# StandeHaas/Hydrodynamic-Limits-of-Active-Particle-Systems-with-Mean-Field-Interactions

Measured on AMD Instinct MI355X. Metric: particle-steps/sec at N=1e5, higher is better.
Workload: dtype f64; 1 GPU; BASELINE config 2: N=100000 particles, L=200000 sites, K=1, reflecting walls, sigma=0.005 (4001-tap table), beta=0.7, dt=0.0125, exclusion on; method=tiles

## Files before the change

hydrodynamic-limits-of-active-particle-systems-with-mean-field-interactions_amd/csrc/aps_hip.hip:

```cpp

#include <hip/hip_runtime.h>
#include <hip/hip_ext.h>
#include <dlfcn.h>
#include <unistd.h>
#include <rccl/rccl.h>
#include <algorithm>
#include <cmath>
#include <cstdint>
#include <cstdio>
#include <cstdlib>
#include <cstring>
#include <numeric>
#include <string>
#include <vector>

#include "aps.h"
#include "aps_common.hpp"
#include "dev_mem.hpp"

namespace {

constexpr uint32_t POS_MASK = 0x07FFFFFFu;
constexpr uint32_t SPIN_BIT = 1u << 27;
constexpr uint32_t BOUND_BIT = 1u << 28;
// ... 1718 lines not shown
#endif
#undef TS_CASE
#undef TS_PICK
}
const void *ts_kernel(bool periodic, bool tab, int RS, bool k1, bool f32 = false) {
    return f32 ? ts_kernel_f<true>(periodic, tab, RS, k1) : ts_kernel_f<false>(periodic, tab, RS, k1);
}
constexpr int TS_RS_CHOICES[] = {1, 2, 3, 4, 5, 6, 7, 8};

int ts_wbytes(const aps_handle *h) { return h->f32 ? 4 : 8; }

void ts_choose_geometry(aps_handle *h) {
    const int L = h->p.L;
    h->ts_RS = 1;
    double best = 1e300;
    for (int rs : TS_RS_CHOICES) {
        const int own = 64 * rs - 4;
        const double wgs = (double)(((int64_t)L + own - 1) / own) * h->E;
        const double miss = std::fabs(wgs - 2.4 * 256.0);
        if (miss < best) { best = miss; h->ts_RS = rs; }
    }
    if ((double)(((int64_t)L + 507) / 508) * h->E > 3.0 * 256.0)
        h->ts_RS = !h->f32 ? 4 : 7;
    int own_even = 0;
    if (h->world == 1 && h->model.field_mode && 3 * h->p.K <= 32 && !(h->p.K == 1 && h->model.immobilize && h->model.k_exit > 0.0)) {
        int cus = 0;
        if (hipDeviceGetAttribute(&cus, hipDeviceAttributeMultiprocessorCount, h->p.device) != hipSuccess || cus <= 0) { (void)hipGetLastError(); cus = 256; }
        const int64_t target = 2LL * cus / std::max(h->E, 1);
        if (target >= 1) {
            const int own = (int)((L + target - 1) / target), rs = (own + 4 + 63) / 64;
            if (own >= 124 && rs <= 8) { h->ts_RS = rs; own_even = own; }
        }
    }
    if (const char *env = std::getenv("APS_TS_R")) { const int r = std::atoi(env); if (ts_kernel(false, true, r, true)) { h->ts_RS = r; own_even = 0; } }
    h->ts_own = own_even ? own_even : 64 * h->ts_RS - 4;
    if (const char *env = std::getenv("APS_TS_OWN")) { const int o = std::atoi(env); if (o >= 32 * h->ts_RS && o <= 64 * h->ts_RS - 4) h->ts_own = o; }
    while (h->ts_own > 32 * h->ts_RS && L > h->ts_own && (L % h->ts_own == 1 || L % h->ts_own == 2)) h->ts_own -= 1;
    h->ts_ntile = (L + h->ts_own - 1) / h->ts_own;
    h->ts_dcap = (int)std::max<int64_t>(2, std::min<int64_t>(2LL * h->p.K * h->ts_own, 2 * h->p.n_particles));
    h->ts_table_in_lds = ts_lds_layout(h->tlen, true, h->ts_RS, h->ts_own, h->p.K, ts_wbytes(h)).total <= 160 * 1024;
    h->ts_lo = (int)((int64_t)h->rank * h->ts_ntile / h->world);
    h->ts_hi = (int)((int64_t)(h->rank + 1) * h->ts_ntile / h->world);
    h->own_lo = h->ts_lo * h->ts_own;
    h->own_hi = std::min(L, h->ts_hi * h->ts_own);
    h->ts_reach = h->model.field_mode ? (h->tlen + 2 + h->ts_own - 1) / h->ts_own : 0;
    h->ts_kx = 1;
    if (h->world > 1) {
        const int reach = std::max(h->ts_reach, 1);
        int own_min = h->ts_ntile, own_max = 0;
        for (int r = 0; r < h->world; ++r) {
            const int n = (int)((int64_t)(r + 1) * h->ts_ntile / h->world) - (int)((int64_t)r * h->ts_ntile / h->world);
            own_min = std::min(own_min, n); own_max = std::max(own_max, n);
        }
        auto fits = [&](int k) { return k * reach <= own_min && own_max + 2 * (k - 1) * reach <= h->ts_ntile; };
        const int64_t budget = std::max<int64_t>(768 / std::max(h->E, 1), (int64_t)own_max + own_max / 4);
        int k = 1;
        while (k < 8 && fits(k + 1) && own_max + 2 * k * reach <= budget) ++k;
        if (h->p.halo_interval > 0) k = h->p.halo_interval;
        else if (const char *env = std::getenv("APS_HALO_INTERVAL")) k = std::max(1, std::atoi(env));
        h->ts_kx = k;
    }
}

TileArgs tile_args(aps_handle *h, bool field_only) {
    TileArgs a{};
    const int par = (int)(h->step & 1), out = field_only ? par : par ^ 1;
    a.L = h->p.L; a.K = h->p.K; a.tlen = h->tlen; a.own = h->ts_own; a.ntile = h->ts_ntile; a.dcap = h->ts_dcap; a.par = par;
    a.dense = h->ntt_on ? h->d_ntt_csig : nullptr; a.dense_rt = h->ntt.Rt; a.dense_m = h->ntt.lc; a.periodic = h->p.periodic;
    a.dense_org = h->ntt.org; a.dense_shard = h->world > 1 ? 1 : 0;
    a.dense_lo = h->world > 1 ? h->own_lo : 0; a.dense_hi = h->world > 1 ? h->own_hi : h->p.L;
    a.tile_lo = h->ts_lo; a.field_only = field_only ? 1 : 0; a.field_mode = h->model.field_mode; a.ens_base = h->model.ens_base; a.E = h->E;
    a.seed_lo = h->model.seed_lo; a.seed_hi = h->model.seed_hi;
    a.model = h->d_model; a.rare = h->d_rare;
    a.ws_in = h->f32 ? (const void *)h->d_wsi[par] : (const void *)h->d_wsb[par];
    a.ws_out = h->f32 ? (void *)h->d_wsi[out] : (void *)h->d_wsb[out];
    a.cell_in = h->d_cell[par]; a.cell_out = h->d_cell[par ^ 1];
    a.dcnt_in = h->d_tdcnt[par]; a.dep_in = h->d_tdep[par]; a.dcnt_out = h->d_tdcnt[par ^ 1]; a.dep_out = h->d_tdep[par ^ 1];
    a.gpart_in = h->d_gpart[par]; a.gpart_out = h->d_gpart[par ^ 1];
    a.stepw = h->d_stepw; a.beta = h->d_beta; a.anchor = h->d_anchor;
    return a;
}

int launch_tile_step(aps_handle *h, bool field_only = false) {
    int rc = field_only ? APS_OK : prof_mark(h, KIND_TILE_STEP);
    if (rc) return rc;
    TileArgs a = tile_args(h, field_only);
    if (h->ntt_on) {
        if (field_only) return fail(h, APS_ERR_STATE, "tiles, convolution: no deposits are ever pending");
        a.tile_lo = 0;
        const dim3 grid((unsigned)td_tiles(a.dense_hi - a.dense_lo), (unsigned)h->E), block(FU_THREADS);
        const void *fn = h->f32 ? (h->p.K == 1 ? reinterpret_cast<const void *>(&tile_dense<true, true>) : reinterpret_cast<const void *>(&tile_dense<false, true>))
                                : (h->p.K == 1 ? reinterpret_cast<const void *>(&tile_dense<true, false>) : reinterpret_cast<const void *>(&tile_dense<false, false>));
        void *args[] = {(void *)&a};
        if (h->profiling && h->prof_dispatch) HIP_TRY(h, hipExtLaunchKernel(fn, grid, block, args, td_lds_bytes(h->p.K), h->stream, h->k_start, h->k_stop, 0));
        else HIP_TRY(h, hipLaunchKernel(fn, grid, block, args, td_lds_bytes(h->p.K), h->stream));
        h->slots_dirty = true; h->field_pending = true; h->ws_view_stale = true;
        return APS_OK;
    }
    int t0 = h->ts_lo, t1 = h->ts_hi;
    if (h->world > 1) {
        if (!field_only && h->halo_age >= h->ts_kx) return fail(h, APS_ERR_STATE, "tiles, sharded: the halo exchange of the last step is missing");
        const int g = (h->ts_kx - 1 - std::min(h->halo_age, h->ts_kx - 1)) * h->ts_reach + (field_only ? 1 : 0);
        t0 = h->p.periodic ? t0 - g : std::max(0, t0 - g);
        t1 = h->p.periodic ? t1 + g : std::min(h->ts_ntile, t1 + g);
    }
    const void *fn = ts_kernel(h->p.periodic != 0, h->ts_table_in_lds, h->ts_RS, h->p.K == 1, h->f32);
    const size_t lds = ts_lds_layout(h->tlen, h->ts_table_in_lds, h->ts_RS, h->ts_own, h->p.K, ts_wbytes(h)).total;
    const void *table_ptr = h->f32 ? (const void *)h->d_table_i : (const void *)h->d_table;
    void *args[] = {(void *)&a, (void *)&table_ptr};
    struct Piece { int lo, hi; } pieces[3];
    int np = 0;
    if (t0 < 0) pieces[np++] = {t0 + h->ts_ntile, h->ts_ntile};
    pieces[np++] = {std::max(t0, 0), std::min(t1, h->ts_ntile)};
    if (t1 > h->ts_ntile) pieces[np++] = {0, t1 - h->ts_ntile};
    for (int i = 0; i < np; ++i) {
        if (pieces[i].hi <= pieces[i].lo) continue;
        a.tile_lo = pieces[i].lo;
        const dim3 grid((unsigned)(pieces[i].hi - pieces[i].lo), (unsigned)h->E), block(FU_THREADS);
        if (!field_only && h->profiling && h->prof_dispatch)
            HIP_TRY(h, hipExtLaunchKernel(fn, grid, block, args, lds, h->stream, h->k_start, h->k_stop, 0));
        else
            HIP_TRY(h, hipLaunchKernel(fn, grid, block, args, lds, h->stream));
    }
    if (!field_only) { h->slots_dirty = true; h->field_pending = true; }
    h->ws_view_stale = true;
    return APS_OK;
}

int launch_ntt_conv(aps_handle *h) {
    const int out = (int)((h->step & 1) ^ 1);
    const NttPlan &pl = h->ntt;
    const unsigned tiles = (unsigned)(((size_t)1 << pl.m) / NTT_TILE);
    const dim3 grid_e(tiles, 2u, (unsigned)(h->E * pl.nb)), grid_p(tiles, 2u, (unsigned)(h->E * pl.np * pl.nb)), block(NTT_THREADS);
    int *const clr = pl.nb > 1 ? h->d_ntt_csig : nullptr;
    void *ws = h->f32 ? (void *)h->d_wsi[out] : (void *)h->d_wsb[out];
    int rc;
    const bool timed = h->profiling && h->prof_dispatch;
#define NTT_STRIDED(AXIS, INV, NP_, GRID, A_, CSIG, WS, FLAG) do { if ((rc = prof_mark(h, KIND_NTT))) return rc; \
        ntt_launch_strided<AXIS, INV, NP_>(A_, GRID, block, h->stream, h->k_start, h->k_stop, timed, pl, h->d_ntt_sig, CSIG, WS, FLAG); } while (0)
#define NTT_ENDS(AXIS, INV, A_, CSIG, WS) do { if (pl.np == 2) NTT_STRIDED(2, INV, 2, grid_e, A_, CSIG, WS, 1); else NTT_STRIDED(AXIS, INV, 1, grid_e, A_, CSIG, WS, 1); } while (0)
    if (h->ntt_fused) {
        NTT_ENDS(2, false, pl.a2, h->d_ntt_csig, nullptr);
        if ((rc = prof_mark(h, KIND_NTT))) return rc;
        APS_K(h, ntt_mid, dim3(1u << pl.a2, 2u, (unsigned)(h->E * pl.np * pl.nb)), dim3(NTT_MID_THREADS), NTT_MID_LDS, pl, h->d_ntt_sig);
        NTT_ENDS(2, true, pl.a2, clr, ws);
        HIP_TRY(h, hipGetLastError());
        h->field_pending = false;
        return APS_OK;
    }
    if (pl.a2 > 0) {
        NTT_ENDS(2, false, pl.a2, h->d_ntt_csig, nullptr);
        NTT_STRIDED(1, false, 1, grid_p, pl.a1, (int *)nullptr, nullptr, 0);
    } else NTT_ENDS(1, false, pl.a1, h->d_ntt_csig, nullptr);
    if ((rc = prof_mark(h, KIND_NTT))) return rc;
    APS_K(h, (ntt_contig<false>), grid_p, block, 0, pl, h->d_ntt_sig);
    if (pl.a2 > 0) {
        NTT_STRIDED(1, true, 1, grid_p, pl.a1, (int *)nullptr, nullptr, 0);
        NTT_ENDS(2, true, pl.a2, clr, ws);
    } else NTT_ENDS(1, true, pl.a1, clr, ws);
#undef NTT_ENDS
#undef NTT_STRIDED
    HIP_TRY(h, hipGetLastError());
    h->field_pending = false;
    return APS_OK;
}

int run_ntt_conv(aps_handle *h) {
    const int rc = launch_ntt_conv(h);
    if (rc) {
        h->field_dirty = true;
        h->field_pending = false;
        (void)hipGetLastError();
        (void)hipMemsetAsync(h->d_ntt_csig, 0, (size_t)h->E * 2 * ((size_t)1 << h->ntt.lc) * 4, h->stream);
        if (h->world > 1) for (int64_t &n : h->n_set) n = -1;
    }
    return rc;
}

void rank_tiles(const aps_handle *h, int r, int &lo, int &hi);

int ntt_setup(aps_handle *h) {
    h->ntt_on = false;
    const char *env = std::getenv("APS_NTT");
    if (env && env[0] == '0') return APS_OK;
    const bool forced = env && env[0] == '1';
    if (!is_tiles(h) || !h->model.field_mode) return APS_OK;
    if (h->ts_table_in_lds && !forced) return APS_OK;
    const int Rt = h->tlen - 1, L = h->p.L;
    const bool shard = h->world > 1;
    int64_t span = (int64_t)L + 2 * Rt;
    if (!shard) {
        if (h->p.periodic ? !(2 * Rt <= L && L >= 4 * TD_SITES) : !(2 * Rt + 64 * h->ts_RS + h->ts_own + 4 < L)) return APS_OK;
    } else {
        const char *kenv = std::getenv("APS_HALO_INTERVAL");
        if (h->p.halo_interval > 1 || (h->p.halo_interval == 0 && kenv && std::atoi(kenv) > 1)) return APS_OK;
        int own_min = L, own_max = 0;
        for (int r = 0; r < h->world; ++r) {
            int lo, hi;
            rank_tiles(h, r, lo, hi);
            const int n = std::min(L, hi * h->ts_own) - lo * h->ts_own;
            own_min = std::min(own_min, n); own_max = std::max(own_max, n);
        }
        span = (int64_t)own_max + 2 * (Rt + TD_HALO);
        if (own_min < Rt + TD_HALO + 1 || (h->p.periodic && span > L)) return APS_OK;
    }
    const int np = h->f32 ? 1 : 2;
    int m, nb = 1, bs = 0;
    if (shard) {
        m = ntt_min_log2(np);
        while (((int64_t)1 << m) < span) ++m;
        if (m > NTT_MAX_LOG2) return APS_OK;
    } else {
        int cap = NTT_MAX_LOG2;
        if (const char *cenv = std::getenv("APS_NTT_MAX_LOG2")) { const int v = std::atoi(cenv); if (v >= 14 && v <= NTT_MAX_LOG2) cap = v; }
        if (!ntt_plan_blocks(L, Rt, np, cap, nb, m, bs)) return APS_OK;
        if ((int64_t)np * h->E * nb > 65535) return APS_OK;
        if (nb > 1 && !forced) return APS_OK;
    }
    if (td_lds_bytes(h->p.K) > 160 * 1024) return APS_OK;
    if (td_lds_bytes(h->p.K) > 48 * 1024) {
        const void *fn = h->f32 ? reinterpret_cast<const void *>(&tile_dense<false, true>) : reinterpret_cast<const void *>(&tile_dense<false, false>);
        if (hipFuncSetAttribute(fn, hipFuncAttributeMaxDynamicSharedMemorySize, (int)td_lds_bytes(h->p.K)) != hipSuccess) { (void)hipGetLastError(); return APS_OK; }
    }
    double wsum = 0.0;
    for (int t = 0; t < h->tlen; ++t) wsum += std::ldexp(h->table[(size_t)t], h->q) * (t ? 2.0 : 1.0);
    if (2.0 * h->p.K * wsum >= 0.5 * (np == 1 ? (double)NTT_PRIMES[0] : (double)NTT_PRIMES[0] * (double)NTT_PRIMES[1])) return APS_OK;
    NttPlan &pl = h->ntt;
    pl.m = m; ntt_split(m, pl.a0, pl.a1, pl.a2); pl.L = L; pl.Rt = Rt; pl.E = h->E; pl.np = np;
    pl.org = shard ? h->own_lo - Rt - TD_HALO : -Rt;
    pl.out_lo = shard ? h->own_lo - TD_HALO : 0;
    pl.out_hi = shard ? h->own_hi + TD_HALO : L;
    if (shard && !h->p.periodic) { pl.out_lo = std::max(pl.out_lo, 0); pl.out_hi = std::min(pl.out_hi, L); }
    pl.nb = nb; pl.bs = nb > 1 ? bs : pl.out_hi - pl.out_lo; pl.lc = m;
    if (nb > 1) while (((int64_t)1 << pl.lc) < (int64_t)(nb - 1) * bs + ((int64_t)1 << m)) ++pl.lc;
    pl.crt_inv = ntt_powmod(NTT_PRIMES[0] % NTT_PRIMES[1], NTT_PRIMES[1] - 2ull, NTT_PRIMES[1]);
    pl.unit = std::ldexp(1.0, -h->q);
    const size_t M = (size_t)1 << m;
    NttTables T[2];
    for (int k = 0; k < np; ++k) ntt_build_tables(m, NTT_PRIMES[k], NTT_ROOTS[k], T[k]);
    const size_t o_wr = 0, o_t1 = o_wr + T[0].wr.size(), o_hi = o_t1 + T[0].t1.size(), o_lo = o_hi + T[0].t2hi.size(), o_what = o_lo + T[0].t2lo.size(),
                 o_whatp = o_what + M, per_prime = o_whatp + M;
    int rc;
    if ((rc = dev_alloc(h, &h->d_ntt_tab, per_prime * np)) || (rc = dev_alloc(h, &h->d_ntt_sig, (size_t)np * h->E * nb * 2 * M)) ||
        (rc = dev_alloc(h, &h->d_ntt_csig, ((size_t)h->E * 2) << pl.lc))) return rc;
    for (int k = 0; k < np; ++k) {
        uint32_t *tb = h->d_ntt_tab + (size_t)k * per_prime;
        HIP_TRY(h, hipMemcpyAsync(tb + o_wr, T[k].wr.data(), T[k].wr.size() * 4, hipMemcpyHostToDevice, h->stream));
        HIP_TRY(h, hipMemcpyAsync(tb + o_t1, T[k].t1.data(), T[k].t1.size() * 4, hipMemcpyHostToDevice, h->stream));
        HIP_TRY(h, hipMemcpyAsync(tb + o_hi, T[k].t2hi.data(), T[k].t2hi.size() * 4, hipMemcpyHostToDevice, h->stream));
        HIP_TRY(h, hipMemcpyAsync(tb + o_lo, T[k].t2lo.data(), T[k].t2lo.size() * 4, hipMemcpyHostToDevice, h->stream));
        NttPrime &pp = pl.pr[k];
        pp.P = NTT_PRIMES[k]; pp.md.P = (double)NTT_PRIMES[k]; pp.md.Pinv = 1.0 / (double)NTT_PRIMES[k];
        pp.wr = tb + o_wr; pp.t1 = tb + o_t1; pp.t2hi = tb + o_hi; pp.t2lo = tb + o_lo; pp.what = tb + o_what; pp.whatp = tb + o_whatp;
    }
    if (np == 1) pl.pr[1] = pl.pr[0];
    const char *fenv = std::getenv("APS_NTT_FUSED");
    h->ntt_fused = pl.a0 == 7 && pl.a1 == 7 && pl.a2 >= 1 && !(fenv && fenv[0] == '0');
    if (h->ntt_fused && hipFuncSetAttribute(reinterpret_cast<const void *>(&ntt_mid), hipFuncAttributeMaxDynamicSharedMemorySize, (int)NTT_MID_LDS) != hipSuccess) {
        (void)hipGetLastError(); h->ntt_fused = false;
    }
    {
        NttPlan ps = pl;
        ps.E = 1; ps.nb = 1;
        std::vector<uint32_t> wext((size_t)np * 2 * M, 0u);
        for (int k = 0; k < np; ++k)
            for (int t = 0; t < h->tlen; ++t) {
                const uint32_t v = (uint32_t)((unsigned long long)std::ldexp(h->table[(size_t)t], h->q) % NTT_PRIMES[k]);
                wext[(size_t)k * 2 * M + (size_t)t] = v;
                if (t && !(h->p.periodic && 2 * t == L)) wext[(size_t)k * 2 * M + M - (size_t)t] = v;
            }
        HIP_TRY(h, hipMemcpyAsync(h->d_ntt_sig, wext.data(), wext.size() * 4, hipMemcpyHostToDevice, h->stream));
        const dim3 grid((unsigned)(M / NTT_TILE), 1u, (unsigned)np), block(NTT_THREADS);
        if (pl.a2 > 0) ntt_launch_strided<2, false, 1>(pl.a2, grid, block, h->stream, nullptr, nullptr, false, ps, h->d_ntt_sig, nullptr, nullptr, 0);
        ntt_launch_strided<1, false, 1>(pl.a1, grid, block, h->stream, nullptr, nullptr, false, ps, h->d_ntt_sig, nullptr, nullptr, 0);
        hipLaunchKernelGGL((ntt_contig<true>), grid, block, 0, h->stream, ps, h->d_ntt_sig);
        HIP_TRY(h, hipGetLastError());
        std::vector<uint32_t> spec(M), specp;
        for (int k = 0; k < np; ++k) {
            HIP_TRY(h, hipMemcpyAsync(spec.data(), h->d_ntt_sig + (size_t)k * 2 * M, M * 4, hipMemcpyDeviceToHost, h->stream));
            HIP_TRY(h, hipStreamSynchronize(h->stream));
            const uint32_t P = NTT_PRIMES[k], minv = ntt_powmod((uint32_t)(M % P), P - 2ull, P);
            for (size_t i = 0; i < M; ++i) spec[i] = ntt_mulmod_u64(spec[i], minv, P);
            HIP_TRY(h, hipMemcpy(h->d_ntt_tab + (size_t)k * per_prime + o_what, spec.data(), M * 4, hipMemcpyHostToDevice));
            if (h->ntt_fused) {
                specp.resize(M);
                auto brev7 = [](size_t v) { size_t r = 0; for (int b = 0; b < 7; ++b) r |= ((v >> b) & 1) << (6 - b); return r; };
                for (size_t k2 = 0; k2 < (M >> 14); ++k2)
                    for (size_t s0 = 0; s0 < 128; ++s0)
                        for (size_t s1 = 0; s1 < 128; ++s1) specp[(k2 << 14) + s0 * 128 + s1] = spec[(k2 << 14) + brev7(s1) * 128 + brev7(s0)];
                HIP_TRY(h, hipMemcpy(h->d_ntt_tab + (size_t)k * per_prime + o_whatp, specp.data(), M * 4, hipMemcpyHostToDevice));
            }
        }
    }
    HIP_TRY(h, hipMemsetAsync(h->d_ntt_sig, 0, (size_t)np * h->E * nb * 2 * M * 4, h->stream));
    HIP_TRY(h, hipStreamSynchronize(h->stream));
    if (h->d_wsi[1] != h->d_wsi[0]) { h->mem.release(h->d_wsi[1]); h->d_wsi[1] = h->d_wsi[0]; }
    if (!h->f32 && h->d_wsb[1] != h->d_wsb[0]) { h->mem.release(h->d_wsb[1]); h->d_wsb[1] = h->d_wsb[0]; }
    if (shard) h->ts_kx = 1;
    h->ntt_on = true;
    return APS_OK;
}

template <bool F32>
const void *tl_kernel_f(bool periodic, int RS, bool k1) {
#define TL_PICK(BC, R) (k1 ? (const void *)&tile_loop<BC, R, true, F32> : (const void *)&tile_loop<BC, R, false, F32>)
#define TL_CASE(R) case R: return periodic ? TL_PICK(1, R) : TL_PICK(0, R);
    if (!F32 && (RS == 8 || (RS == 7 && !k1))) return nullptr;
#ifdef APS_DEV_RS
    switch (RS) { TL_CASE(APS_DEV_RS) default: return nullptr; }
#else
    if constexpr (F32) { if (RS == 8) return periodic ? TL_PICK(1, 8) : TL_PICK(0, 8); }
    switch (RS) {
        TL_CASE(1) TL_CASE(2) TL_CASE(3) TL_CASE(4) TL_CASE(5) TL_CASE(6)
        case 7: return k1 ? (periodic ? (const void *)&tile_loop<1, 7, true, F32> : (const void *)&tile_loop<0, 7, true, F32>)
                          : (F32 ? (periodic ? (const void *)&tile_loop<1, 7, false, true> : (const void *)&tile_loop<0, 7, false, true>) : nullptr);
        default: return nullptr;
    }
#endif
#undef TL_CASE
#undef TL_PICK
}
const void *tl_kernel(const aps_handle *h) {
    return h->f32 ? tl_kernel_f<true>(h->p.periodic != 0, h->ts_RS, h->p.K == 1) : tl_kernel_f<false>(h->p.periodic != 0, h->ts_RS, h->p.K == 1);
}

int loop_prepare(aps_handle *h) {
    if (h->loop_state != -2) return APS_OK;
    h->loop_state = 0;
    auto no = [&](const char *why) { h->loop_why = why; return APS_OK; };
    if (!is_tiles(h)) return no("not the tiles formulation");
    if (h->world != 1) return no("sharded handle");
    if (h->ntt_on) return no("field updated by the exact convolution");
    if (!h->ts_table_in_lds) return no("weight table beyond LDS");
    if (!h->model.field_mode) return no("global mean field");
    if (h->p.K == 1 && h->model.immobilize && h->model.k_exit > 0.0) return no("particles can leave the system (one cell per site)");
    if (3 * h->p.K > 32) return no("site capacity above 10");
    if (h->p.L - (int64_t)(h->ts_ntile - 1) * h->ts_own < 3) return no("last tile shorter than three sites");
#ifdef APS_STAMPS
    return no("diagnostic build");
#endif
    const void *fn = tl_kernel(h);
    if (!fn) return no("no kernel for this frame");
    const int64_t need_per_cu = ((int64_t)h->ts_ntile * h->E + h->num_cu - 1) / h->num_cu;
    h->loop_seg = 0;
    size_t lds_total = 0;
    for (int seg : {256, 192, 128, TL_SEG_MIN}) {
        const TlLds lay = tl_lds_layout(h->tlen, h->ts_RS, h->ts_own, h->p.K, ts_wbytes(h), seg);
        if (lay.total > 160 * 1024) continue;
        if (128 / (int)((lay.total + 1279) / 1280) >= need_per_cu) { h->loop_seg = seg; lds_total = lay.total; break; }
    }
    if (!h->loop_seg) return no("more tiles than the device keeps resident at once (LDS)");
    if (lds_total > 48 * 1024 && hipFuncSetAttribute(fn, hipFuncAttributeMaxDynamicSharedMemorySize, (int)lds_total) != hipSuccess) { (void)hipGetLastError(); return no("hipFuncSetAttribute failed"); }
    int per_cu = 0;
    if (hipOccupancyMaxActiveBlocksPerMultiprocessor(&per_cu, fn, FU_THREADS, lds_total) != hipSuccess) { (void)hipGetLastError(); return no("occupancy query failed"); }
    if (need_per_cu > std::min(per_cu, 8)) return no("more tiles than the device keeps resident at once");
    h->loop_drec = (h->ts_dcap / 16 + 1) * 16;
    h->loop_rec = (h->loop_drec + 6 * h->p.K + 15) / 16 * 16;
    int rc;
    if ((rc = dev_alloc(h, &h->d_xrec, (size_t)2 * h->E * h->ts_ntile * h->loop_rec)) || (rc = dev_alloc(h, &h->d_abort, 4))) return rc;
    HIP_TRY(h, h->mem.alloc_host_mapped(&h->h_abort, &h->h_abort_dev, 16));
    h->h_abort[0] = 0u;
    h->loop_tag = 0;
    h->loop_state = 1;
    return APS_OK;
}

int launch_tile_loop(aps_handle *h, int64_t n) {
    LoopArgs la{};
    la.a = tile_args(h, false);
    la.a.tile_lo = 0;
    la.step0 = (unsigned long long)h->step;
    la.nsteps = (int)n;
    if ((uint64_t)h->loop_tag + (uint64_t)n + 2 > 0xFFFFFFF0ull) {
        HIP_TRY(h, hipMemsetAsync(h->d_xrec, 0, (size_t)2 * h->E * h->ts_ntile * h->loop_rec * sizeof(unsigned long long), h->stream));
        h->loop_tag = 0;
    }
    la.tag0 = h->loop_tag;
    h->loop_tag += (uint32_t)n + 1u;
    la.rec = h->loop_rec; la.drec = h->loop_drec; la.xrec = h->d_xrec; la.seg = h->loop_seg;
    la.abort_dev = h->d_abort; la.abort_host = h->h_abort_dev;
    la.timeout_ticks = 5000000ull;
    if (const char *env = std::getenv("APS_LOOP_TIMEOUT_MS")) la.timeout_ticks = (unsigned long long)std::max(1, std::atoi(env)) * 100000ull;
#ifdef APS_LOOP_DEBUG
    static uint32_t *dbg = nullptr;
    if (!dbg) (void)hipMalloc(reinterpret_cast<void **>(&dbg), (size_t)64 * 3 * h->p.L * 4);
    (void)hipMemsetAsync(dbg, 0xEE, (size_t)64 * 3 * h->p.L * 4, h->stream);
    la.dbg = n <= 64 ? dbg : nullptr;
    h->loop_dbg = dbg; h->loop_dbg_n = (int)n;
#endif
    if (std::getenv("APS_LOOP_TEST_ABORT")) HIP_TRY(h, hipMemsetAsync(h->d_abort, 1, 4, h->stream));
    {
        unsigned stall = 0u;
        if (const char *env = std::getenv("APS_LOOP_TEST_STALL")) {
            int st_tile = -1, st_it = 0;
            if (std::sscanf(env, "%d:%d", &st_tile, &st_it) == 2 && st_tile >= 0 && st_tile < h->ts_ntile && st_it >= 0 && st_it < 0xFFFF)
                stall = ((unsigned)(st_tile + 1) << 16) | (unsigned)st_it;
        }
        if (stall != h->loop_stall) {
            HIP_TRY(h, hipMemcpyAsync(h->d_abort + 1, &stall, 4, hipMemcpyHostToDevice, h->stream));
            HIP_TRY(h, hipStreamSynchronize(h->stream));
            h->loop_stall = stall;
        }
    }
    const void *fn = tl_kernel(h);
    const size_t lds = tl_lds_layout(h->tlen, h->ts_RS, h->ts_own, h->p.K, ts_wbytes(h), h->loop_seg).total;
    const void *table_ptr = h->f32 ? (const void *)h->d_table_i : (const void *)h->d_table;
    void *args[] = {(void *)&la, (void *)&table_ptr};
    const dim3 grid((unsigned)h->ts_ntile, (unsigned)h->E), block(FU_THREADS);
    if (h->loop_timed) {
        for (hipEvent_t &ev : h->loop_ev) if (!ev) HIP_TRY(h, hipEventCreate(&ev));
        HIP_TRY(h, hipExtLaunchKernel(fn, grid, block, args, lds, h->stream, h->loop_ev[0], h->loop_ev[1], 0));
    } else
        HIP_TRY(h, hipLaunchKernel(fn, grid, block, args, lds, h->stream));
    return APS_OK;
}

struct HaloSeg { size_t off, bytes; int array; };

void halo_segments(const aps_handle *h, int owner_lo_tile, int owner_hi_tile, int side, bool recv, std::vector<HaloSeg> &out) {
    const int L = h->p.L, K = h->p.K, own = h->ts_own;
    const int s_lo = owner_lo_tile * own, s_hi = std::min(L, owner_hi_tile * own);
    if (h->ntt_on) {
        const int reach = h->ntt.Rt + TD_HALO;
        const size_t M = (size_t)1 << h->ntt.m;
        const int p0 = !recv ? (side == 0 ? s_lo - 1 : s_hi - reach) - h->ntt.org
                             : (side == 0 ? h->own_hi - 1 : h->own_lo - reach) - h->ntt.org;
        for (int e = 0; e < h->E; ++e) {
            const int c0 = side == 0 ? s_lo : s_hi - 3, c1 = side == 0 ? s_lo + 3 : s_hi;
            out.push_back({((size_t)e * L + c0) * K * 4, (size_t)(c1 - c0) * K * 4, 0});
            for (int sg = 0; sg < 2; ++sg) out.push_back({(((size_t)e * 2 + sg) * M + (size_t)p0) * 4, (size_t)(reach + 1) * 4, 4});
        }
        return;
    }
    const int nt = std::min(h->ts_kx * h->ts_reach, owner_hi_tile - owner_lo_tile);
    const int64_t gs = (int64_t)(h->ts_kx - 1) * h->ts_reach * own;
    for (int e = 0; e < h->E; ++e) {
        const int64_t g1 = std::min<int64_t>(s_hi, (int64_t)owner_hi_tile * own - gs);
        const int c0 = side == 0 ? s_lo : (int)std::max<int64_t>(s_lo, g1 - 3);
        const int c1 = side == 0 ? (int)std::min<int64_t>(s_hi, s_lo + gs + 3) : s_hi;
        const int w0 = side == 0 ? s_lo : (int)std::max<int64_t>(s_lo, g1 - 2);
        const int w1 = side == 0 ? (int)std::min<int64_t>(s_hi, s_lo + gs + 2) : s_hi;
        const int t0 = side == 0 ? owner_lo_tile : owner_hi_tile - nt, t1 = t0 + nt;
        out.push_back({((size_t)e * L + c0) * K * 4, (size_t)(c1 - c0) * K * 4, 0});
        if (h->model.field_mode) {
            out.push_back({((size_t)e * L + w0) * 2 * ts_wbytes(h), (size_t)(w1 - w0) * 2 * ts_wbytes(h), 1});
            out.push_back({((size_t)e * h->ts_ntile + t0) * 4, (size_t)(t1 - t0) * 4, 2});
            out.push_back({((size_t)e * h->ts_ntile + t0) * h->ts_dcap * 4, (size_t)(t1 - t0) * h->ts_dcap * 4, 3});
        }
    }
}

char *halo_array(aps_handle *h, int array, int buf) {
    switch (array) {
        case 0: return reinterpret_cast<char *>(h->d_cell[buf]);
        case 1: return h->f32 ? reinterpret_cast<char *>(h->d_wsi[buf]) : reinterpret_cast<char *>(h->d_wsb[buf]);
        case 2: return reinterpret_cast<char *>(h->d_tdcnt[buf]);
        case 3: return reinterpret_cast<char *>(h->d_tdep[buf]);
        default: return reinterpret_cast<char *>(h->d_ntt_csig);
    }
}

void rank_tiles(const aps_handle *h, int r, int &lo, int &hi) {
    lo = (int)((int64_t)r * h->ts_ntile / h->world);
    hi = (int)((int64_t)(r + 1) * h->ts_ntile / h->world);
}

void halo_peers(const aps_handle *h, int &left, int &right) {
    left = h->rank - 1; right = h->rank + 1;
    if (h->p.periodic) { left = (left + h->world) % h->world; right %= h->world; }
    else { if (right >= h->world) right = -1; }
}

int halo_setup(aps_handle *h) {
    int left, right, lo, hi;
    halo_peers(h, left, right);
    for (int side = 0; side < 2; ++side) {
        for (int recv = 0; recv < 2; ++recv) {
            std::vector<HaloSeg> segs;
            if (!recv) halo_segments(h, h->ts_lo, h->ts_hi, side, false, segs);
            else {
                const int peer = side == 0 ? right : left;
                if (peer < 0) continue;
                rank_tiles(h, peer, lo, hi);
                halo_segments(h, lo, hi, side, true, segs);
            }
            std::vector<HaloSegD> tab;
            size_t off = 0;
            for (const HaloSeg &g : segs) {
                if (!g.bytes) continue;
                tab.push_back({(unsigned long long)g.off, (unsigned long long)off, (unsigned)g.bytes, g.array});
                off += (g.bytes + 15) / 16 * 16;
            }
            HaloSegD **dseg = recv ? &h->d_halo_seg_recv[side] : &h->d_halo_seg_send[side];
            char **dmsg = recv ? &h->d_halo_recv[side] : &h->d_halo_send[side];
            (recv ? h->halo_nseg_recv[side] : h->halo_nseg_send[side]) = (int)tab.size();
            (recv ? h->halo_bytes_recv[side] : h->halo_bytes_send[side]) = off;
            int rc;
            if ((rc = dev_alloc(h, dseg, tab.size())) || (rc = dev_alloc(h, dmsg, off))) return rc;
            HIP_TRY(h, hipMemcpyAsync(*dseg, tab.data(), tab.size() * sizeof(HaloSegD), hipMemcpyHostToDevice, h->stream));
        }
    }
    HIP_TRY(h, hipStreamSynchronize(h->stream));
    return APS_OK;
}

int halo_launch(aps_handle *h, int side, bool unpack) {
    const int buf = (int)((h->step & 1) ^ 1);
    const int nseg = unpack ? h->halo_nseg_recv[side] : h->halo_nseg_send[side];
    if (!nseg) return APS_OK;
    hipLaunchKernelGGL(halo_move, dim3((unsigned)(nseg * HALO_BPS)), dim3(256), 0, h->stream,
                       unpack ? h->d_halo_seg_recv[side] : h->d_halo_seg_send[side], halo_array(h, 0, buf), halo_array(h, 1, buf),
                       halo_array(h, 2, buf), halo_array(h, 3, buf), halo_array(h, HALO_ADD, buf), unpack ? h->d_halo_recv[side] : h->d_halo_send[side], unpack ? 1 : 0);
    HIP_TRY(h, hipGetLastError());
    return APS_OK;
}

unsigned halo_expected(const aps_handle *h) {
    int left, right;
    halo_peers(h, left, right);
    return (right >= 0 && h->halo_nseg_recv[0] ? 1u : 0u) | (left >= 0 && h->halo_nseg_recv[1] ? 2u : 0u);
}

bool halo_due(const aps_handle *h) { return h->world > 1 && h->halo_age + 1 == h->ts_kx; }

bool halo_prepacked(const aps_handle *h) { return h->ntt_on && h->world > 1 && !h->ipc_on && !h->comm; }

int halo_exchange_rccl(aps_handle *h) {
    int left, right, rc;
    halo_peers(h, left, right);
    if (left >= 0 && (rc = halo_launch(h, 0, false))) return rc;
    if (right >= 0 && (rc = halo_launch(h, 1, false))) return rc;
    ncclResult_t nr = g_rccl.GroupStart();
    if (nr == ncclSuccess && left >= 0 && h->halo_bytes_send[0]) nr = g_rccl.Send(h->d_halo_send[0], h->halo_bytes_send[0], ncclUint8, left, h->comm, h->stream);
    if (nr == ncclSuccess && right >= 0 && h->halo_bytes_send[1]) nr = g_rccl.Send(h->d_halo_send[1], h->halo_bytes_send[1], ncclUint8, right, h->comm, h->stream);
    if (nr == ncclSuccess && right >= 0 && h->halo_bytes_recv[0]) nr = g_rccl.Recv(h->d_halo_recv[0], h->halo_bytes_recv[0], ncclUint8, right, h->comm, h->stream);
    if (nr == ncclSuccess && left >= 0 && h->halo_bytes_recv[1]) nr = g_rccl.Recv(h->d_halo_recv[1], h->halo_bytes_recv[1], ncclUint8, left, h->comm, h->stream);
    const ncclResult_t ge = g_rccl.GroupEnd();
    if (nr == ncclSuccess) nr = ge;
    if (nr != ncclSuccess) return fail(h, APS_ERR_HIP, std::string("halo exchange (ncclSend/ncclRecv): ") + g_rccl.GetErrorString(nr));
    if (right >= 0 && (rc = halo_launch(h, 0, true))) return rc;
    if (left >= 0 && (rc = halo_launch(h, 1, true))) return rc;
    h->halo_got = halo_expected(h);
    return APS_OK;
}

int halo_exchange_ipc(aps_handle *h) {
    int left, right;
    halo_peers(h, left, right);
    const int buf = (int)((h->step & 1) ^ 1), par = (int)(h->ipc_seq & 1u);
    const unsigned tag = h->ipc_seq + 1u;
    HaloPushArgs pu{};
    HaloPullArgs pl{};
    const int peer_of_side[2] = {left, right};
    for (int side = 0; side < 2; ++side) {
        if (peer_of_side[side] >= 0 && h->halo_nseg_send[side]) {
            pu.segs[side] = h->d_halo_seg_send[side]; pu.nseg[side] = h->halo_nseg_send[side];
            pu.dst[side] = h->ipc_peer[side] + h->ipc_peer_off[side][par];
            pu.flag[side] = reinterpret_cast<unsigned long long *>(h->ipc_peer[side] + (size_t)(par * 2 + side) * 64);
        }
        const int from = side == 0 ? right : left;
        if (from >= 0 && h->halo_nseg_recv[side]) {
            pl.segs[side] = h->d_halo_seg_recv[side]; pl.nseg[side] = h->halo_nseg_recv[side];
            pl.src[side] = h->ipc_land + h->ipc_land_off[par][side];
            pl.flag[side] = reinterpret_cast<const unsigned long long *>(h->ipc_land + (size_t)(par * 2 + side) * 64);
        }
    }
    pu.done = h->d_ipc_done; pu.tag = tag;
    pl.tag = tag; pl.err_host = h->h_ipc_err_dev;
    pl.timeout_ticks = 20ull * 100000000ull;
    if (const char *env = std::getenv("APS_HALO_TIMEOUT_MS")) pl.timeout_ticks = (unsigned long long)std::max(1, std::atoi(env)) * 100000ull;
    char *a0 = halo_array(h, 0, buf), *a1 = halo_array(h, 1, buf), *a2 = halo_array(h, 2, buf), *a3 = halo_array(h, 3, buf), *a4 = halo_array(h, HALO_ADD, buf);
    const unsigned nbu = (unsigned)(pu.nseg[0] + pu.nseg[1]) * HALO_BPS, nbl = (unsigned)(pl.nseg[0] + pl.nseg[1]) * HALO_BPS;
    if (nbu) hipLaunchKernelGGL(halo_push, dim3(nbu), dim3(256), 0, h->stream, pu, a0, a1, a2, a3, a4);
    if (nbl) hipLaunchKernelGGL(halo_pull, dim3(nbl), dim3(256), 0, h->stream, pl, a0, a1, a2, a3, a4);
    HIP_TRY(h, hipGetLastError());
    h->ipc_seq += 1u;
    h->halo_got = halo_expected(h);
    return APS_OK;
}

int flush_field(aps_handle *h) {
    if (!is_tiles(h) || !h->field_pending) return APS_OK;
    if (h->ntt_on) return fail(h, APS_ERR_STATE, "tiles, convolution on a site range: the step's convolution runs in aps_commit, after the halo exchange");
    const int cur = (int)(h->step & 1);
    if (h->model.field_mode) {
        int rc = launch_tile_step(h, true);
        if (rc) return rc;
    }
    HIP_TRY(h, hipMemsetAsync(h->d_tdcnt[cur], 0, (size_t)h->E * h->ts_ntile * 4, h->stream));
    h->field_pending = false;
    return APS_OK;
}

int sync_slots(aps_handle *h) {
    if (!is_tiles(h)) return APS_OK;
    int rc = flush_field(h);
    if (rc) return rc;
    const int cur = (int)(h->step & 1);
    h->d_ws = h->d_wsb[cur];
    const int L = h->p.L;
    if (h->f32 && h->model.field_mode && h->ws_view_stale) {
        const size_t n = (size_t)h->E * L;
        hipLaunchKernelGGL(ws_to_double, dim3((unsigned)((n + 255) / 256)), dim3(256), 0, h->stream, h->d_wsi[cur], h->d_wsb[cur], n, std::ldexp(1.0, -h->q));
        HIP_TRY(h, hipGetLastError());
        HIP_TRY(h, hipStreamSynchronize(h->stream));
        h->ws_view_stale = false;
    }
    if (!h->slots_dirty) return APS_OK;
    const int s_lo = h->world > 1 ? h->own_lo : 0, s_hi = h->world > 1 ? h->own_hi : L;
    if (h->world > 1)
        hipLaunchKernelGGL(mark_away, dim3((unsigned)(((size_t)h->E * h->Npad + 255) / 256)), dim3(256), 0, h->stream, h->d_src, (size_t)h->E * h->Npad);
    if (s_hi > s_lo)
        hipLaunchKernelGGL(cells_to_slots, dim3((unsigned)((s_hi - s_lo + 255) / 256), (unsigned)h->E), dim3(256), 0, h->stream,
                           h->d_cell[cur], h->d_slot_of, h->d_src, h->d_occ_site, L, h->p.K, (long long)h->N, (int)h->Npad, s_lo, s_hi);
    hipLaunchKernelGGL(derive_slots, dim3((unsigned)(h->Npad / 256), (unsigned)h->E), dim3(256), 0, h->stream,
                       h->d_src, h->d_sp8, h->d_tinfo, (int)h->Npad, (int)h->ntiles);
    long long *gs = h->d_gsum + (size_t)cur * 2 * h->E;
    HIP_TRY(h, hipMemsetAsync(gs, 0, (size_t)2 * h->E * sizeof(long long), h->stream));
    hipLaunchKernelGGL(tile_parts, dim3((unsigned)h->ts_ntile, (unsigned)h->E), dim3(256), 0, h->stream,
                       h->d_cell[cur], h->d_gpart[cur], gs, L, h->p.K, h->ts_own, h->ts_ntile);
    HIP_TRY(h, hipGetLastError());
    HIP_TRY(h, hipStreamSynchronize(h->stream));
    h->slots_dirty = false;
    h->plan_dirty = true;
    return APS_OK;
}
// ... 1341 lines not shown
```

hydrodynamic-limits-of-active-particle-systems-with-mean-field-interactions_amd/csrc/tile_loop.hpp:

```cpp
#pragma once

constexpr int TL_SEG_MIN = 88;
constexpr int TL_NG = 2;
#ifndef TL_MIN_WAVES
#define TL_MIN_WAVES 2
#endif
constexpr int TL_ABORT = 31;

struct LoopArgs {
    TileArgs a;
    unsigned long long step0;
    int nsteps;
    uint32_t tag0;
    int rec, drec;
    int seg;
    unsigned long long *xrec;
    unsigned *abort_dev, *abort_host;
    unsigned long long timeout_ticks;
#ifdef APS_LOOP_DEBUG
    uint32_t *dbg;
#endif
};

struct TlLds { size_t seg, cells, cells2, props, occ, misc, plist, fw, fs, tab, total; };
__host__ __device__ inline TlLds tl_lds_layout(int tlen, int RS, int own, int K, int wbytes, int seg) {
    TlLds l;
    const size_t TS = 64 * (size_t)RS, ncell = (TS + 2) * K;
    auto up = [](size_t v, size_t a) { return (v + a - 1) / a * a; };
    l.seg = 0;
    l.cells = l.seg + (size_t)FU_WAVES * 4 * (seg + 4) * sizeof(uint32_t);
    l.cells2 = up(l.cells + ncell * 4, 8);
    l.props = up(l.cells2 + (K == 1 ? 0 : ncell * 4), 8);
    l.occ = up(l.props + TS * K, 8);
    l.misc = up(l.occ + TS + 2, 8);
    l.plist = l.misc + 128;
    l.fw = up(l.plist + TS * (size_t)K * 8, 16);
    l.fs = l.fw + TS * wbytes;
    l.tab = up(l.fs + TS * wbytes, 16);
    l.total = l.tab + (size_t)ts_table_chunks(tlen, RS, own, wbytes) * 1024;
    return l;
}

typedef __attribute__((address_space(1))) unsigned long long tl_gu64;
typedef __attribute__((address_space(1))) unsigned tl_gu32;

__device__ __forceinline__ void tl_store_granule(unsigned long long *p, uint32_t tag, uint32_t word) {
    __hip_atomic_store((tl_gu64 *)p, ((unsigned long long)tag << 32) | word, __ATOMIC_RELAXED, __HIP_MEMORY_SCOPE_AGENT);
}
__device__ __forceinline__ unsigned long long tl_load_granule(const unsigned long long *p) {
    return __hip_atomic_load((tl_gu64 *)p, __ATOMIC_RELAXED, __HIP_MEMORY_SCOPE_AGENT);
}

__device__ __forceinline__ void tl_lds_add(double *p, double v) { unsafeAtomicAdd(p, v); }
__device__ __forceinline__ void tl_lds_add(int *p, int v) { atomicAdd(p, v); }

template <int BC, int RS, bool K1, bool F32>
__global__ __launch_bounds__(FU_THREADS, TL_MIN_WAVES) void tile_loop(const LoopArgs la, const void *__restrict__ table_v) {
    using W = typename TsField<F32>::w_t;
    using WS = typename TsField<F32>::ws_t;
    constexpr int SH = TsField<F32>::SH, WB = (int)sizeof(W);
    constexpr bool TAB_LDS = true;
    const TileArgs &a = la.a;
    const W *__restrict__ table_g = reinterpret_cast<const W *>(table_v);
    constexpr int TS = 64 * RS, NOLD = (TS + FU_THREADS - 1) / FU_THREADS;
    constexpr int NSLOT = 16, GB = FU_WAVES * 4;
    const int SEG = la.seg;
    extern __shared__ double lds[];
    const int L = a.L, K = K1 ? 1 : a.K, OWN = a.own;
    const TlLds lay = tl_lds_layout(a.tlen, RS, OWN, K, WB, la.seg);
    char *lds_c = reinterpret_cast<char *>(lds);
    uint32_t *seg_all = reinterpret_cast<uint32_t *>(lds_c + lay.seg);
    uint32_t *cellL = reinterpret_cast<uint32_t *>(lds_c + lay.cells);
    uint32_t *cellN = reinterpret_cast<uint32_t *>(lds_c + lay.cells2);
    uint8_t *propL = reinterpret_cast<uint8_t *>(lds_c + lay.props);
    uint8_t *occL = reinterpret_cast<uint8_t *>(lds_c + lay.occ);
    int *misc = reinterpret_cast<int *>(lds_c + lay.misc);
    uint2 *plist = reinterpret_cast<uint2 *>(lds_c + lay.plist);
    W *fieldW = reinterpret_cast<W *>(lds_c + lay.fw), *fieldS = reinterpret_cast<W *>(lds_c + lay.fs);
    W *tab = reinterpret_cast<W *>(lds_c + lay.tab);
    const int t = threadIdx.x, lane = t & 63, wave = __builtin_amdgcn_readfirstlane(t >> 6), e = blockIdx.y;
    const int tile = (int)blockIdx.x;
    const int own0 = tile * OWN, own_n = min(OWN, L - own0), nfr = own_n + 4;
    const int x0 = own0 - 2;
    const int x0c = max(x0, 0), x1c = min(x0 + nfr - 1, L - 1);
    const int Rt = a.tlen - 1;
    if (__hip_atomic_load((tl_gu32 *)la.abort_dev, __ATOMIC_RELAXED, __HIP_MEMORY_SCOPE_AGENT)) {
        if (t == 0) __hip_atomic_store(la.abort_host, 1u, __ATOMIC_RELAXED, __HIP_MEMORY_SCOPE_SYSTEM);
        return;
    }
    int n_iter = la.nsteps;
    {
        const unsigned stall = la.abort_dev[1];
        if (stall && (int)(stall >> 16) - 1 == tile && e == 0) n_iter = min(n_iter, (int)(stall & 0xFFFFu));
    }
    const uint32_t *__restrict__ cell_e = a.cell_in + (size_t)e * L * K;
    const WS *__restrict__ ws_e = reinterpret_cast<const WS *>(a.ws_in) + (size_t)e * L;
    const uint32_t *__restrict__ dcnt_e = a.dcnt_in + (size_t)e * a.ntile;
    const uint32_t *__restrict__ dep_e = a.dep_in + (size_t)e * a.ntile * a.dcap;
    uint32_t tbase = 0;
    {
        typedef __attribute__((address_space(3))) W lds_w;
        tbase = (uint32_t)(size_t)(lds_w *)tab;
    }
    if (t < 32) misc[t] = 0;
    {
        const int nchunk = ts_table_chunks(a.tlen, RS, OWN, WB);
        const char *srct = reinterpret_cast<const char *>(table_g) + lane * 16;
        for (int c = wave; c < nchunk; c += FU_WAVES) {
            const uint32_t m0v = (uint32_t)__builtin_amdgcn_readfirstlane((int)(tbase + (uint32_t)c * 1024u));
            asm volatile("s_mov_b32 m0, %0\n\tglobal_load_lds_dwordx4 %1, off" :: "s"(m0v), "v"(srct + c * 1024) : "memory");
        }
    }
    const double beta = a.beta[e];
    auto frame_site = [&](int i) -> int {
        if (i < -1 || i > nfr) return -1;
        int s = x0 + i;
        if (BC == 1) { s %= L; if (s < 0) s += L; return s; }
        return (s < 0 || s >= L) ? -1 : s;
    };
    const int ncell = (TS + 2) * K;
    for (int c = t; c < ncell; c += FU_THREADS) {
        const int s = frame_site(c / K - 1);
        const uint32_t v = cell_e[(unsigned)max(s, 0) * (unsigned)K + (unsigned)(c % K)];
        cellL[c] = s >= 0 ? v : CELL_EMPTY;
        if (!K1) cellN[c] = CELL_EMPTY;
    }
#pragma unroll
    for (int r = 0; r < NOLD; ++r) {
        const int xi = r * FU_THREADS + t;
        if (xi < TS) {
            const int s = xi < nfr ? frame_site(xi) : -1;
            WS o = ws_e[(unsigned)max(s, 0)];
            if (s < 0) { o.x = 0; o.y = 0; }
            fieldW[xi] = o.x; fieldS[xi] = o.y;
        }
    }
    for (int i = t; i < (TS * K + 3) / 4; i += FU_THREADS) reinterpret_cast<uint32_t *>(propL)[i] = 0u;
    int b0 = 0, nbk = 0;
    if (BC == 0) {
        b0 = max(0, x0c - Rt - 1) / OWN;
        nbk = min(L - 1, x1c + Rt + 1) / OWN - b0 + 1;
    } else {
        const int lo = x0 - Rt - 1, hi = x0 + nfr - 1 + Rt + 1;
        if (hi - lo + 1 >= L) { b0 = 0; nbk = a.ntile; }
        else {
            const int lom = ((lo % L) + L) % L, him = ((hi % L) + L) % L;
            const int blo = lom / OWN, bhi = him / OWN;
            b0 = blo;
            nbk = (lom <= him) ? bhi - blo + 1 : (a.ntile - blo) + bhi + 1;
            if (nbk > a.ntile) { b0 = 0; nbk = a.ntile; }
        }
    }
    const bool wall = BC == 0 && ((x0c + 1 <= Rt) || (L - x1c <= Rt));
    const bool mirror_ok = 2 * Rt + TS + OWN + 4 < L;
    const int sub = lane >> 4, slot = lane & (NSLOT - 1);
    const uint32_t tlen8 = (uint32_t)a.tlen << SH, L8 = (uint32_t)L << SH;
    uint32_t x8[RS];
#pragma unroll
    for (int r = 0; r < RS; ++r) {
        int s = x0 + r * 64 + lane;
        if (BC == 1) { s %= L; if (s < 0) s += L; } else s = min(max(s, 0), L - 1);
        x8[r] = ((uint32_t)s + TS_BIAS) << SH;
    }
    const int nb_l = tile > 0 ? tile - 1 : (BC == 1 ? a.ntile - 1 : -1), nb_r = tile + 1 < a.ntile ? tile + 1 : (BC == 1 ? 0 : -1);
    const size_t rec_e = (size_t)e * a.ntile;
    const int null_site = x0c;
    const uint32_t tb = tbase;
    uint32_t *dep_o = a.dep_out + ((size_t)e * a.ntile + tile) * a.dcap;
    uint32_t *cell_o = a.cell_out + (size_t)e * L * K;
    const int ngroups = (nbk + GB - 1) / GB;
    const int npass = (wall && mirror_ok) ? 2 : 1;
    auto append = [&](bool occ, int pos, int k, uint32_t cw, int *counter) {
        const unsigned long long mm = __ballot(occ);
        const int cnt_u = __popcll(mm);
        int base = 0;
        if (lane == 0 && cnt_u) base = atomicAdd(counter, cnt_u);
        base = __builtin_amdgcn_readfirstlane(base);
        if (occ) plist[base + __builtin_amdgcn_mbcnt_hi((uint32_t)(mm >> 32), __builtin_amdgcn_mbcnt_lo((uint32_t)mm, 0u))] = make_uint2((uint32_t)pos | ((uint32_t)k << 16), cw);
    };
    asm volatile("s_waitcnt vmcnt(0)" ::: "memory");
    __syncthreads();
    for (int i = t; i < TS + 2; i += FU_THREADS) {
        int n = 0;
        for (int k = 0; k < K; ++k) n += cellL[i * K + k] != CELL_EMPTY;
        occL[i] = (uint8_t)n;
    }
    for (int c0 = 0; c0 < ncell; c0 += FU_THREADS) {
        const int c = c0 + t;
        const int pos = K1 ? c - 1 : c / K - 1, k = K1 ? 0 : c - (pos + 1) * K;
        const uint32_t cw = c < ncell ? cellL[c] : CELL_EMPTY;
        append(cw != CELL_EMPTY && pos >= 0 && pos < nfr, pos, k, cw, misc + 2);
    }
    __syncthreads();

#ifdef APS_LOOP_STAMPS
    unsigned long long st_acc[12] = {0, 0, 0, 0, 0, 0, 0, 0, 0, 0, 0, 0}, st_t0 = __builtin_amdgcn_s_memtime();
    const unsigned long long st_begin = st_t0;
#define TLSTAMP(k) { const unsigned long long t1_ = __builtin_amdgcn_s_memtime(); st_acc[k] += t1_ - st_t0; st_t0 = t1_; }
#else
#define TLSTAMP(k)
#endif
    unsigned long long xg[TL_NG], xh = 0;
#pragma unroll
    for (int g = 0; g < TL_NG; ++g) xg[g] = 0;
    const int h_side = lane >> 5, h_i = lane & 31;
    const int h_nb = h_side ? nb_r : nb_l;
    const bool h_act = wave == FU_WAVES - 1 && h_i < 3 * K && h_nb >= 0;
    auto bucket_of = [&](int j, bool &ok) -> int {
        const int bi = j * GB + sub * FU_WAVES + wave;
        ok = j < ngroups && bi < nbk;
        int b = b0 + (ok ? bi : 0);
        if (b >= a.ntile) b -= a.ntile;
        return b;
    };
    for (int it = 0; it < n_iter; ++it) {
        const unsigned long long step = la.step0 + (unsigned long long)it;
        const uint32_t tag_in = la.tag0 + (uint32_t)it, tag_out = tag_in + 1u;
        const bool first = it == 0, last = it + 1 == la.nsteps;
        const unsigned long long *rec_in = la.xrec + ((size_t)((it + 1) & 1) * a.E * a.ntile + rec_e) * la.rec;
        unsigned long long *rec_out = la.xrec + ((size_t)(it & 1) * a.E * a.ntile + rec_e + tile) * la.rec;
        int *dcount = misc + (it & 1), *pcount = misc + 2 + (it & 1);
        bool gave_up = false;
        const int n0 = *pcount;
        uint2 mine = make_uint2(0u, CELL_EMPTY);
        uint32_t rx[4] = {0u, 0u, 0u, 0u};
        if (t < n0) {
            mine = plist[t];
            philox4x32_10((uint32_t)step, (uint32_t)(step >> 32), mine.y & CELL_ID, (uint32_t)(a.ens_base + e), a.seed_lo, a.seed_hi, rx);
        }
        TLSTAMP(2)
        auto spin_check = [&](unsigned &spins, unsigned long long &t_w) -> bool {
            __builtin_amdgcn_s_sleep(1);
            if ((++spins & 63u) != 0u) return false;
            const bool other = __hip_atomic_load((tl_gu32 *)la.abort_dev, __ATOMIC_RELAXED, __HIP_MEMORY_SCOPE_AGENT) != 0;
            const unsigned long long now = __builtin_amdgcn_s_memrealtime();
            if (!t_w) t_w = now;
            if (!other && now - t_w <= la.timeout_ticks) return false;
            if (!other && lane == 0) {
                __hip_atomic_store((tl_gu32 *)la.abort_dev, 1u, __ATOMIC_RELAXED, __HIP_MEMORY_SCOPE_AGENT);
                __hip_atomic_store(la.abort_host, 1u, __ATOMIC_RELAXED, __HIP_MEMORY_SCOPE_SYSTEM);
            }
            gave_up = true;
            return true;
        };
        auto wait_granule = [&](const unsigned long long *p, bool active) -> uint32_t {
            unsigned long long x = 0, t_w = 0;
            for (unsigned spins = 0;;) {
                if (active) x = tl_load_granule(p);
                if (!__ballot(active && (uint32_t)(x >> 32) != tag_in)) break;
                if (spin_check(spins, t_w)) break;
            }
            return (uint32_t)x;
        };
        if (!first) {
            unsigned long long t_w = 0;
            for (unsigned spins = 0;;) {
                bool bad = false;
#pragma unroll
                for (int g = 0; g < TL_NG; ++g) {
                    bool ok;
                    const int b = bucket_of(g, ok);
                    if (ok && (uint32_t)(xg[g] >> 32) != tag_in) {
                        xg[g] = tl_load_granule(rec_in + (size_t)b * la.rec + slot);
                        bad |= (uint32_t)(xg[g] >> 32) != tag_in;
                    }
                }
                if (h_act && (uint32_t)(xh >> 32) != tag_in) {
                    xh = tl_load_granule(rec_in + (size_t)h_nb * la.rec + la.drec + (h_side ? 0 : 3 * K) + h_i);
                    bad |= (uint32_t)(xh >> 32) != tag_in;
                }
                if (!__ballot(bad)) break;
                if (spin_check(spins, t_w)) break;
            }
            if (wave == FU_WAVES - 1 && !gave_up) {
                const uint32_t v = h_act ? (uint32_t)xh : CELL_EMPTY;
                const int hs = h_i / K, hk = h_i - hs * K, pos = (h_side ? own_n + 2 : -1) + hs;
                if (h_act) cellL[(h_side ? (own_n + 3) * K : 0) + h_i] = v;
                const unsigned long long mo = __ballot(h_act && v != CELL_EMPTY);
                if (h_i < 3 * K && hk == 0 && h_nb >= 0) occL[pos + 1] = (uint8_t)__popcll((mo >> (h_side * 32 + hs * K)) & ((1ull << K) - 1ull));
                const bool hp = h_act && v != CELL_EMPTY && pos >= 0 && pos < nfr;
                const unsigned long long mh = __ballot(hp);
                if (hp) plist[n0 + __builtin_amdgcn_mbcnt_hi((uint32_t)(mh >> 32), __builtin_amdgcn_mbcnt_lo((uint32_t)mh, 0u))] = make_uint2((uint32_t)pos | ((uint32_t)hk << 16), v);
                if (lane == 0) misc[4 + (it & 1)] = __popcll(mh);
            }
        }
        TLSTAMP(0)
        W accP[RS], accM[RS], accF[RS], accWi[RS], accSi[RS];
#pragma unroll
        for (int r = 0; r < RS; ++r) accP[r] = accM[r] = accF[r] = accWi[r] = accSi[r] = 0;
        uint32_t *shl = seg_all;
        const int CAP = (FU_WAVES * 4 * (SEG + 4) / 4) & ~3;
        unsigned long long *shcnt = reinterpret_cast<unsigned long long *>(misc + 8 + 2 * (it & 1));
        auto sweep_now = [&](unsigned long long m, const uint32_t word, const int cls) {
            while (m) {
                const int src_lane = __builtin_ctzll(m);
                m &= m - 1;
                const uint32_t e1 = (uint32_t)__builtin_amdgcn_readlane((int)word, src_lane);
                if (BC == 0) {
                    if (cls == 0) ts_one_abs<RS, 0, F32>(e1, x8, tb, accP);
                    else if (cls == 1) ts_one_abs<RS, 0, F32>(e1, x8, tb, accM);
                    else if (cls == 2) ts_one_abs<RS, 1, F32>(e1, x8, tb, accF);
                    else ts_image_group<TAB_LDS, RS, F32>(make_uint4(e1, DEP_NULL | ((uint32_t)x0c + TS_BIAS), DEP_NULL | ((uint32_t)x0c + TS_BIAS), DEP_NULL | ((uint32_t)x0c + TS_BIAS)),
                                                          x8, tb, table_g, tlen8, L8, accWi, accSi);
                } else {
                    const uint4 q = make_uint4(e1, DEP_NULL | ((uint32_t)null_site + TS_BIAS), DEP_NULL | ((uint32_t)null_site + TS_BIAS), DEP_NULL | ((uint32_t)null_site + TS_BIAS));
                    if (cls == 0) ts_group<1, TAB_LDS, RS, 0, F32>(q, x8, tb, table_g, tlen8, L8, accP);
                    else if (cls == 1) ts_group<1, TAB_LDS, RS, 0, F32>(q, x8, tb, table_g, tlen8, L8, accM);
                    else ts_group<1, TAB_LDS, RS, 1, F32>(q, x8, tb, table_g, tlen8, L8, accF);
                }
            }
        };
#pragma unroll 1
        for (int j = 0; j < ngroups && !gave_up; ++j) {
            bool ok;
            const int b = bucket_of(j, ok);
            uint32_t cnt = 0u;
            if (first) { cnt = min(dcnt_e[(unsigned)b], (uint32_t)a.dcap); if (!ok) cnt = 0u; }
            const unsigned long long *rb = rec_in + (size_t)b * la.rec;
            bool active = ok;
#pragma unroll 1
            for (int page = 0;; ++page) {
                uint32_t en = DEP_NULL;
                bool valid = false, more = false;
                if (first) {
                    const uint32_t k0 = (uint32_t)page * NSLOT;
                    en = dep_e[(unsigned)b * (unsigned)a.dcap + min(k0 + slot, (uint32_t)a.dcap - 1u)];
                    valid = k0 + slot < cnt; more = k0 + NSLOT < cnt;
                } else if (__ballot(active)) {
                    if (page == 0 && j < TL_NG) {
                        unsigned long long x = xg[0];
#pragma unroll
                        for (int g = 1; g < TL_NG; ++g) if (j == g) x = xg[g];
                        en = (uint32_t)x;
                    } else {
                        en = wait_granule(rb + min(page * NSLOT + slot, la.drec - 1), active);
                        if (gave_up) break;
                    }
                    valid = active && en != DEP_NULL;
                    const unsigned long long mv = __ballot(valid);
                    more = active && ((mv >> (sub * 16 + 15)) & 1ull) && (page + 1) * NSLOT < la.drec;
                }
                const uint32_t en_ = en + TS_BIAS;
                if (!wall) {
                    const int cw = (int)((en_ >> 27) & 3u) - 1, cs = (int)(en_ >> 29) - 2;
                    const bool cP = valid && cw != 0 && cw == cs, cM = valid && cw != 0 && cw != cs, cF = valid && cw == 0;
                    const unsigned long long kP = __ballot(cP), kM = __ballot(cM), kF = __ballot(cF);
                    const unsigned long long add = (unsigned long long)__popcll(kP) | ((unsigned long long)__popcll(kM) << 16) | ((unsigned long long)__popcll(kF) << 32);
                    if (add) {
                        unsigned long long base = 0;
                        if (lane == 0) base = atomicAdd(shcnt, add);
                        const uint32_t blo = (uint32_t)__builtin_amdgcn_readfirstlane((int)(uint32_t)base), bhi = (uint32_t)__builtin_amdgcn_readfirstlane((int)(uint32_t)(base >> 32));
                        const bool room = (int)(blo & 0xFFFFu) + __popcll(kP) <= CAP && (int)(blo >> 16) + __popcll(kM) <= CAP && (int)(bhi & 0xFFFFu) + __popcll(kF) <= CAP;
#define TL_POOL(MASK, COND, WORD, CLS, BASE) { \
                        const int i_ = (int)(BASE) + (int)__builtin_amdgcn_mbcnt_hi((uint32_t)((MASK) >> 32), __builtin_amdgcn_mbcnt_lo((uint32_t)(MASK), 0u)); \
                        if ((COND) && (room || i_ < CAP)) shl[(CLS) * CAP + i_] = (WORD); \
                        if (!room) { const unsigned long long o_ = __ballot((COND) && i_ >= CAP); if (o_) sweep_now(o_, (WORD), (CLS)); } }
                        TL_POOL(kP, cP, en_, 0, blo & 0xFFFFu) TL_POOL(kM, cM, en_, 1, blo >> 16) TL_POOL(kF, cF, en_, 2, bhi & 0xFFFFu)
#undef TL_POOL
                    }
                    active = more;
                    if (!__ballot(active)) break;
                    continue;
                }
                const int dp = (int)(en & POS_MASK), cw = (int)((en_ >> 27) & 3u) - 1, cs = (int)(en_ >> 29) - 2;
                const bool img_l = valid && wall && (x0c + dp + 1 <= Rt), img_r = valid && wall && (2 * L - 1 - x1c - dp <= Rt);
                const bool cP = cw != 0 && cw == cs, cM = cw != 0 && cw != cs, cF = cw == 0;
                const bool im = img_l || img_r;
                const bool pl = valid && (mirror_ok || !im), mi = im && mirror_ok, ii = valid && im && !mirror_ok;
                const uint32_t mir = (en_ & ~POS_MASK) | (uint32_t)((int)TS_BIAS + (img_l ? -1 - dp : 2 * L - 1 - dp));
                const unsigned long long kP = __ballot(pl && cP), kM = __ballot(pl && cM), kF = __ballot(pl && cF);
                const unsigned long long gP = __ballot(mi && cP), gM = __ballot(mi && cM), gF = __ballot(mi && cF), kI = __ballot(ii);
                const unsigned long long add = (unsigned long long)(__popcll(kP) + __popcll(gP)) | ((unsigned long long)(__popcll(kM) + __popcll(gM)) << 16) |
                                               ((unsigned long long)(__popcll(kF) + __popcll(gF)) << 32) | ((unsigned long long)__popcll(kI) << 48);
                if (add) {
                    unsigned long long base = 0;
                    if (lane == 0) base = atomicAdd(shcnt, add);
                    const uint32_t blo = (uint32_t)__builtin_amdgcn_readfirstlane((int)(uint32_t)base), bhi = (uint32_t)__builtin_amdgcn_readfirstlane((int)(uint32_t)(base >> 32));
#define TL_POOL(MASK, COND, WORD, CLS, BASE) { \
                    const int i_ = (int)(BASE) + (int)__builtin_amdgcn_mbcnt_hi((uint32_t)((MASK) >> 32), __builtin_amdgcn_mbcnt_lo((uint32_t)(MASK), 0u)); \
                    if ((COND) && i_ < CAP) shl[(CLS) * CAP + i_] = (WORD); \
                    const unsigned long long o_ = __ballot((COND) && i_ >= CAP); \
                    if (o_) sweep_now(o_, (WORD), (CLS)); }
                    TL_POOL(kP, (pl && cP), en_, 0, blo & 0xFFFFu) TL_POOL(gP, (mi && cP), mir, 0, (blo & 0xFFFFu) + __popcll(kP))
                    TL_POOL(kM, (pl && cM), en_, 1, blo >> 16) TL_POOL(gM, (mi && cM), mir, 1, (blo >> 16) + __popcll(kM))
                    TL_POOL(kF, (pl && cF), en_, 2, bhi & 0xFFFFu) TL_POOL(gF, (mi && cF), mir, 2, (bhi & 0xFFFFu) + __popcll(kF))
                    TL_POOL(kI, ii, en_, 3, bhi >> 16)
#undef TL_POOL
                }
                active = more;
                if (!__ballot(active)) break;
            }
        }
        if (gave_up && lane == 0) misc[TL_ABORT] = 1;
        TLSTAMP(8)
        __syncthreads();
        TLSTAMP(9)
        if (misc[TL_ABORT]) return;
        {
            const unsigned long long tot = *shcnt;
            const int nP = min((int)(tot & 0xFFFFu), CAP), nM = min((int)((tot >> 16) & 0xFFFFu), CAP), nF = min((int)((tot >> 32) & 0xFFFFu), CAP),
                      nI = min((int)(tot >> 48), CAP);
            const uint32_t nullw = DEP_NULL | ((uint32_t)null_site + TS_BIAS);
            int rot = wave;
#define TL_SHARED(CLS, N, CALL4) { \
            const int ng_ = ((N) + 3) >> 2; \
            const uint4 *l4 = reinterpret_cast<const uint4 *>(shl + (CLS) * CAP); \
            int g = rot & 3; \
            uint4 q = l4[min(g, CAP / 4 - 1)]; \
            _Pragma("unroll 1") for (; g < ng_; g += FU_WAVES) { \
                const uint4 qn = l4[min(g + FU_WAVES, CAP / 4 - 1)]; \
                if (4 * g + 3 >= (N)) {                         \
                    if (4 * g + 1 >= (N)) q.y = nullw; \
                    if (4 * g + 2 >= (N)) q.z = nullw; \
                    q.w = nullw; } \
                CALL4; \
                q = qn; } \
            rot = (rot - ng_) & 3; }
            if (BC == 1) {
                TL_SHARED(0, nP, (ts_group<1, TAB_LDS, RS, 0, F32>(q, x8, tb, table_g, tlen8, L8, accP)))
                TL_SHARED(1, nM, (ts_group<1, TAB_LDS, RS, 0, F32>(q, x8, tb, table_g, tlen8, L8, accM)))
                TL_SHARED(2, nF, (ts_group<1, TAB_LDS, RS, 1, F32>(q, x8, tb, table_g, tlen8, L8, accF)))
            } else {
                TL_SHARED(0, nP, (ts_group<0, TAB_LDS, RS, 0, F32>(q, x8, tb, table_g, tlen8, L8, accP)))
                TL_SHARED(1, nM, (ts_group<0, TAB_LDS, RS, 0, F32>(q, x8, tb, table_g, tlen8, L8, accM)))
                TL_SHARED(2, nF, (ts_group<0, TAB_LDS, RS, 1, F32>(q, x8, tb, table_g, tlen8, L8, accF)))
            }
#undef TL_SHARED
            if (nI) {
                const uint32_t nulli = DEP_NULL | ((uint32_t)x0c + TS_BIAS);
                const uint4 *l4 = reinterpret_cast<const uint4 *>(shl + 3 * CAP);
#pragma unroll 1
                for (int g = rot & 3; g < (nI + 3) >> 2; g += FU_WAVES) {
                    uint4 q = l4[g];
                    if (4 * g + 1 >= nI) q.y = nulli;
                    if (4 * g + 2 >= nI) q.z = nulli;
                    if (4 * g + 3 >= nI) q.w = nulli;
                    ts_image_group<TAB_LDS, RS, F32>(q, x8, tb, table_g, tlen8, L8, accWi, accSi);
                }
            }
        }
        TLSTAMP(10)
#pragma unroll
        for (int r = 0; r < RS; ++r) {
            const W dw = (accP[r] + accM[r]) + accWi[r], ds = ((accP[r] - accM[r]) + accF[r]) + accSi[r];
            if (dw != 0) tl_lds_add(&fieldW[r * 64 + lane], dw);
            if (ds != 0) tl_lds_add(&fieldS[r * 64 + lane], ds);
        }
        TLSTAMP(11)
        __syncthreads();
        TLSTAMP(7)
        {
            const Model M = *a.model;
            const int n_part = n0 + misc[4 + (it & 1)];
            auto propose_one = [&](const uint2 pc, const uint32_t (&x)[4]) {
                const int pos = (int)(pc.x & 0xFFFFu), k = (int)(pc.x >> 16);
                const int s = frame_site(pos);
                const bool anch = a.anchor ? a.anchor[s] != 0 : false;
                propL[pos * K + k] = decide_proposal(M, anch, s, (pc.y & CELL_PLUS) ? 1 : -1, (pc.y & CELL_BOUND) != 0,
                                                     clip_field((double)fieldS[pos], (double)fieldW[pos]), beta, occL[pos + 1], occL[pos], occL[pos + 2], x);
            };
            if (t < n_part) {
                if (t >= n0) {
                    mine = plist[t];
                    philox4x32_10((uint32_t)step, (uint32_t)(step >> 32), mine.y & CELL_ID, (uint32_t)(a.ens_base + e), a.seed_lo, a.seed_hi, rx);
                }
                propose_one(mine, rx);
            }
            for (int j = FU_THREADS + t; j < n_part; j += FU_THREADS) {
                const uint2 pc = plist[j];
                uint32_t x[4];
                philox4x32_10((uint32_t)step, (uint32_t)(step >> 32), pc.y & CELL_ID, (uint32_t)(a.ens_base + e), a.seed_lo, a.seed_hi, x);
                propose_one(pc, x);
            }
        }
        __syncthreads();
        TLSTAMP(3)
        auto rank_at = [&](int j, uint32_t id) -> int {
            int n = 0;
            for (int k = 0; k < K; ++k) {
                const uint32_t cl_ = cellL[j * K + k], cr_ = cellL[(j + 2) * K + k];
                const int el = propL[(j - 1) * K + k] & 7, er = propL[(j + 1) * K + k] & 7;
                n += (cl_ != CELL_EMPTY && (el == EV_RIGHT || el == EV_FWD) && (cl_ & CELL_ID) < id);
                n += (cr_ != CELL_EMPTY && er == EV_LEFT && (cr_ & CELL_ID) < id);
            }
            return n;
        };
        auto cap_at = [&](int j) -> int { const int c = K - (int)occL[j + 1]; return c < 1 ? 1 : (c > 32 ? 32 : c); };
        auto put_deposit = [&](int kd, uint32_t d) { if (last) dep_o[kd] = d; else tl_store_granule(rec_out + kd, tag_out, d); };
        auto log_exit = [&](const uint32_t c, const int s) {
            const TileRare R = *a.rare;
            const unsigned kx = atomicAdd(&R.n_exit[e], 1u);
            if ((int)kx < R.exit_cap) {
                double *row = R.exit_log + ((size_t)e * R.exit_cap + kx) * 3;
                row[0] = (double)step; row[1] = (double)s; row[2] = (double)(c & CELL_ID);
            }
            R.src[(size_t)e * R.Npad + R.slot_of[(size_t)e * R.N + (c & CELL_ID)]] =
                (uint32_t)s | DEAD_BIT | ((c & CELL_PLUS) ? SPIN_BIT : 0u) | ((c & CELL_BOUND) ? BOUND_BIT : 0u);
        };
        uint32_t newc[NOLD];
        int newn[NOLD];
#pragma unroll
        for (int r = 0; r < NOLD; ++r) {
            newc[r] = CELL_EMPTY; newn[r] = 0;
            const int xi = r * FU_THREADS + t;
            if (xi < 2 || xi >= 2 + own_n || xi >= TS) continue;
            const int s = frame_site(xi);
            if constexpr (K1) {
                const uint32_t cm2 = cellL[xi - 1], cm1 = cellL[xi], c0 = cellL[xi + 1], cp1 = cellL[xi + 2], cp2 = cellL[xi + 3];
                const int pm2 = propL[xi - 2] & 7, pm1 = propL[xi - 1] & 7, p0 = propL[xi] & 7, pp1 = propL[xi + 1] & 7, pp2 = xi + 2 < TS ? propL[xi + 2] & 7 : 0;
                const bool from_l2 = cm2 != CELL_EMPTY && (pm2 == EV_RIGHT || pm2 == EV_FWD);
                const bool from_l1 = cm1 != CELL_EMPTY && (pm1 == EV_RIGHT || pm1 == EV_FWD);
                const bool from_r1 = cp1 != CELL_EMPTY && pp1 == EV_LEFT;
                const bool from_r2 = cp2 != CELL_EMPTY && pp2 == EV_LEFT;
                uint32_t c = c0;
                if (c != CELL_EMPTY) {
                    const int sgn = (c & CELL_PLUS) ? 1 : -1;
                    uint32_t d0 = 0, d1 = 0;
                    int nd = 0;
                    bool stays = true;
                    if (p0 == EV_LEFT || p0 == EV_RIGHT || p0 == EV_FWD) {
                        const bool left = p0 == EV_LEFT;
                        const int rivals = left ? (int)(from_l2 && (cm2 & CELL_ID) < (c & CELL_ID)) + (int)(false)
                                                : (int)(from_r2 && (cp2 & CELL_ID) < (c & CELL_ID));
                        if (rivals < 1) {
                            stays = false;
                            d0 = deposit(s, -1, -sgn); d1 = deposit(frame_site(left ? xi - 1 : xi + 1), 1, sgn); nd = 2;
                        }
                    } else if (p0 == EV_BIND) c |= CELL_BOUND;
                    else if (p0 == EV_UNBIND) c &= ~CELL_BOUND;
                    else if (p0 == EV_FLIP) { c ^= CELL_PLUS; d0 = deposit(s, 0, -2 * sgn); nd = 1; }
                    if (stays) { newc[r] = c; newn[r] = 1; }
                    if (nd) {
                        const int kd = atomicAdd(dcount, nd);
                        if (kd + nd <= a.dcap) { put_deposit(kd, d0); if (nd == 2) put_deposit(kd + 1, d1); }
                    }
                }
                if (from_l1 && !(from_r1 && (cp1 & CELL_ID) < (cm1 & CELL_ID))) { newc[r] = cm1; newn[r] += 1; }
                if (from_r1 && !(from_l1 && (cm1 & CELL_ID) < (cp1 & CELL_ID))) { newc[r] = cp1; newn[r] += 1; }
                continue;
            }
            uint32_t *outN = cellN + (xi + 1) * K;
            int n_out = 0;
            auto emit = [&](uint32_t c) { if (K1) newc[r] = c; else outN[n_out] = c; ++n_out; };
            for (int k = 0; k < K; ++k) {
                uint32_t c = cellL[(xi + 1) * K + k];
                if (c == CELL_EMPTY) continue;
                const int ev = propL[xi * K + k] & 7, sgn = (c & CELL_PLUS) ? 1 : -1;
                uint32_t d0 = 0, d1 = 0;
                int nd = 0;
                bool stays = true;
                if (ev == EV_LEFT || ev == EV_RIGHT || ev == EV_FWD) {
                    const int j = ev == EV_LEFT ? xi - 1 : xi + 1;
                    if (rank_at(j, c & CELL_ID) < cap_at(j)) {
                        stays = false;
                        d0 = deposit(s, -1, -sgn); d1 = deposit(frame_site(j), 1, sgn); nd = 2;
                    }
                } else if (ev == EV_BIND) c |= CELL_BOUND;
                else if (ev == EV_UNBIND) c &= ~CELL_BOUND;
                else if (ev == EV_FLIP) { c ^= CELL_PLUS; d0 = deposit(s, 0, -2 * sgn); nd = 1; }
                else if (ev == EV_EXIT) { stays = false; log_exit(c, s); d0 = deposit(s, -1, -sgn); nd = 1; }
                if (stays) emit(c);
                if (nd) {
                    const int kd = atomicAdd(dcount, nd);
                    if (kd + nd <= a.dcap) { put_deposit(kd, d0); if (nd == 2) put_deposit(kd + 1, d1); }
                }
            }
            const int cap = cap_at(xi);
            for (int k = 0; k < K; ++k) {
                const uint32_t cl_ = cellL[xi * K + k], cr_ = cellL[(xi + 2) * K + k];
                const int el = propL[(xi - 1) * K + k] & 7, er = propL[(xi + 1) * K + k] & 7;
                if (cl_ != CELL_EMPTY && (el == EV_RIGHT || el == EV_FWD) && rank_at(xi, cl_ & CELL_ID) < cap) emit(cl_);
                if (cr_ != CELL_EMPTY && er == EV_LEFT && rank_at(xi, cr_ & CELL_ID) < cap) emit(cr_);
            }
            if (!K1) for (int k = n_out; k < K; ++k) outN[k] = CELL_EMPTY;
            newn[r] = n_out;
        }
        __syncthreads();
        TLSTAMP(4)
        const int count = min(*dcount, a.dcap);
        int *pnext = misc + 2 + ((it + 1) & 1);
#pragma unroll
        for (int r = 0; r < NOLD; ++r) {
            const int xi = r * FU_THREADS + t;
            const bool mine_site = !(xi < 2 || xi >= 2 + own_n || xi >= TS);
            const int io = xi - 2;
            for (int k = 0; k < K; ++k) {
                uint32_t c = CELL_EMPTY;
                if (mine_site) {
                    c = K1 ? newc[r] : cellN[(xi + 1) * K + k];
                    cellL[(xi + 1) * K + k] = c;
                    if (last) cell_o[(unsigned)frame_site(xi) * (unsigned)K + (unsigned)k] = c;
                    else {
                        if (io < 3) tl_store_granule(rec_out + la.drec + io * K + k, tag_out, c);
                        if (io >= own_n - 3) tl_store_granule(rec_out + la.drec + 3 * K + (io - (own_n - 3)) * K + k, tag_out, c);
                    }
                }
                if (!last) append(mine_site && c != CELL_EMPTY, xi, k, c, pnext);
            }
            if (mine_site) {
                occL[xi + 1] = (uint8_t)newn[r];
                if (last) {
                    WS f; f.x = fieldW[xi]; f.y = fieldS[xi];
                    reinterpret_cast<WS *>(a.ws_out)[(size_t)e * L + (unsigned)frame_site(xi)] = f;
                }
            }
        }
        if (!last && t < NSLOT) {
            const int idx = count + t;
            if (idx < (count / NSLOT + 1) * NSLOT && idx < la.drec) tl_store_granule(rec_out + idx, tag_out, DEP_NULL);
        }
        for (int i = t; i < (TS * K + 3) / 4; i += FU_THREADS) reinterpret_cast<uint32_t *>(propL)[i] = 0u;
        if (t == 0) {
            misc[(it + 1) & 1] = 0;
            misc[2 + (it & 1)] = 0; misc[4 + (it & 1)] = 0;
            misc[8 + 2 * (it & 1)] = 0; misc[9 + 2 * (it & 1)] = 0;
            if (last) {
                a.dcnt_out[(size_t)e * a.ntile + tile] = (uint32_t)count;
                if (tile == 0 && e == 0) a.stepw[(a.par + la.nsteps) & 1] = la.step0 + (unsigned long long)la.nsteps;
            }
        }
        if (!last) {
            const unsigned long long *rn = la.xrec + ((size_t)(it & 1) * a.E * a.ntile + rec_e) * la.rec;
#pragma unroll
            for (int g = 0; g < TL_NG; ++g) {
                bool ok;
                const int b = bucket_of(g, ok);
                xg[g] = ok ? tl_load_granule(rn + (size_t)b * la.rec + slot) : 0ull;
            }
            xh = h_act ? tl_load_granule(rn + (size_t)h_nb * la.rec + la.drec + (h_side ? 0 : 3 * K) + h_i) : 0ull;
        }
        TLSTAMP(5)
        __syncthreads();
    }
#ifdef APS_LOOP_STAMPS
    if (lane == 0 && tile < 512 && e == 0) {
        unsigned long long *o = a.rare->stamps + ((size_t)tile * FU_WAVES + wave) * 16;
        for (int k = 0; k < 12; ++k) o[k] = st_acc[k];
        o[6] = __builtin_amdgcn_s_memtime() - st_begin;
        o[1] = st_acc[8] + st_acc[9] + st_acc[10] + st_acc[11];
    }
#endif
}
```

Baseline: 8.233 billion particle-steps/s.

## Double-buffer tile cells, defer halo wait, and specialize out image-term path

Ping-pongs the cell and occupancy arrays in LDS between iterations, so the update and write-back phases merge and one block barrier per step goes away. The halo-granule spin wait now runs after the deposit scan instead of before it, and per-group waits take their prefetched value. A new IMG template parameter compiles out the mirror-image accumulators and image-group work when the tile geometry never needs them, with a device-side abort if host and kernel disagree. This costs more LDS (cellN is now always allocated), which may lower occupancy, and the ordering across the removed barrier needs care.

```diff
diff --git a/hydrodynamic-limits-of-active-particle-systems-with-mean-field-interactions_amd/csrc/aps_hip.hip b/hydrodynamic-limits-of-active-particle-systems-with-mean-field-interactions_amd/csrc/aps_hip.hip
--- a/hydrodynamic-limits-of-active-particle-systems-with-mean-field-interactions_amd/csrc/aps_hip.hip
+++ b/hydrodynamic-limits-of-active-particle-systems-with-mean-field-interactions_amd/csrc/aps_hip.hip
@@ -2044,8 +2044,9 @@
 }
 
 template <bool F32>
-const void *tl_kernel_f(bool periodic, int RS, bool k1) {
-#define TL_PICK(BC, R) (k1 ? (const void *)&tile_loop<BC, R, true, F32> : (const void *)&tile_loop<BC, R, false, F32>)
+const void *tl_kernel_f(bool periodic, int RS, bool k1, bool img) {
+#define TL_PICK_K(BC, R, IM) (k1 ? (const void *)&tile_loop<BC, R, true, F32, IM> : (const void *)&tile_loop<BC, R, false, F32, IM>)
+#define TL_PICK(BC, R) (BC == 0 && img ? TL_PICK_K(0, R, true) : TL_PICK_K(BC, R, false))
 #define TL_CASE(R) case R: return periodic ? TL_PICK(1, R) : TL_PICK(0, R);
     if (!F32 && (RS == 8 || (RS == 7 && !k1))) return nullptr;
 #ifdef APS_DEV_RS
@@ -2054,16 +2055,23 @@
     if constexpr (F32) { if (RS == 8) return periodic ? TL_PICK(1, 8) : TL_PICK(0, 8); }
     switch (RS) {
         TL_CASE(1) TL_CASE(2) TL_CASE(3) TL_CASE(4) TL_CASE(5) TL_CASE(6)
-        case 7: return k1 ? (periodic ? (const void *)&tile_loop<1, 7, true, F32> : (const void *)&tile_loop<0, 7, true, F32>)
-                          : (F32 ? (periodic ? (const void *)&tile_loop<1, 7, false, true> : (const void *)&tile_loop<0, 7, false, true>) : nullptr);
+        case 7:
+            if (k1) return periodic ? (const void *)&tile_loop<1, 7, true, F32, false>
+                                    : (img ? (const void *)&tile_loop<0, 7, true, F32, true> : (const void *)&tile_loop<0, 7, true, F32, false>);
+            if constexpr (F32) return periodic ? (const void *)&tile_loop<1, 7, false, true, false>
+                                               : (img ? (const void *)&tile_loop<0, 7, false, true, true> : (const void *)&tile_loop<0, 7, false, true, false>);
+            return nullptr;
         default: return nullptr;
     }
 #endif
 #undef TL_CASE
 #undef TL_PICK
+#undef TL_PICK_K
 }
 const void *tl_kernel(const aps_handle *h) {
-    return h->f32 ? tl_kernel_f<true>(h->p.periodic != 0, h->ts_RS, h->p.K == 1) : tl_kernel_f<false>(h->p.periodic != 0, h->ts_RS, h->p.K == 1);
+    const bool periodic = h->p.periodic != 0;
+    const bool img = !periodic && !tl_mirror_ok(h->tlen, h->p.L, h->ts_RS, h->ts_own);
+    return h->f32 ? tl_kernel_f<true>(periodic, h->ts_RS, h->p.K == 1, img) : tl_kernel_f<false>(periodic, h->ts_RS, h->p.K == 1, img);
 }
 
 int loop_prepare(aps_handle *h) {
diff --git a/hydrodynamic-limits-of-active-particle-systems-with-mean-field-interactions_amd/csrc/tile_loop.hpp b/hydrodynamic-limits-of-active-particle-systems-with-mean-field-interactions_amd/csrc/tile_loop.hpp
--- a/hydrodynamic-limits-of-active-particle-systems-with-mean-field-interactions_amd/csrc/tile_loop.hpp
+++ b/hydrodynamic-limits-of-active-particle-systems-with-mean-field-interactions_amd/csrc/tile_loop.hpp
@@ -22,7 +22,7 @@
 #endif
 };
 
-struct TlLds { size_t seg, cells, cells2, props, occ, misc, plist, fw, fs, tab, total; };
+struct TlLds { size_t seg, cells, cells2, props, occ, occ2, misc, plist, fw, fs, tab, total; };
 __host__ __device__ inline TlLds tl_lds_layout(int tlen, int RS, int own, int K, int wbytes, int seg) {
     TlLds l;
     const size_t TS = 64 * (size_t)RS, ncell = (TS + 2) * K;
@@ -30,9 +30,10 @@
     l.seg = 0;
     l.cells = l.seg + (size_t)FU_WAVES * 4 * (seg + 4) * sizeof(uint32_t);
     l.cells2 = up(l.cells + ncell * 4, 8);
-    l.props = up(l.cells2 + (K == 1 ? 0 : ncell * 4), 8);
+    l.props = up(l.cells2 + ncell * 4, 8);
     l.occ = up(l.props + TS * K, 8);
-    l.misc = up(l.occ + TS + 2, 8);
+    l.occ2 = up(l.occ + TS + 2, 8);
+    l.misc = up(l.occ2 + TS + 2, 8);
     l.plist = l.misc + 128;
     l.fw = up(l.plist + TS * (size_t)K * 8, 16);
     l.fs = l.fw + TS * wbytes;
@@ -41,6 +42,8 @@
     return l;
 }
 
+__host__ __device__ inline bool tl_mirror_ok(int tlen, int L, int RS, int own) { return 2 * (long long)(tlen - 1) + 64 * RS + own + 4 < (long long)L; }
+
 typedef __attribute__((address_space(1))) unsigned long long tl_gu64;
 typedef __attribute__((address_space(1))) unsigned tl_gu32;
 
@@ -54,7 +57,7 @@
 __device__ __forceinline__ void tl_lds_add(double *p, double v) { unsafeAtomicAdd(p, v); }
 __device__ __forceinline__ void tl_lds_add(int *p, int v) { atomicAdd(p, v); }
 
-template <int BC, int RS, bool K1, bool F32>
+template <int BC, int RS, bool K1, bool F32, bool IMG>
 __global__ __launch_bounds__(FU_THREADS, TL_MIN_WAVES) void tile_loop(const LoopArgs la, const void *__restrict__ table_v) {
     using W = typename TsField<F32>::w_t;
     using WS = typename TsField<F32>::ws_t;
@@ -70,10 +73,11 @@
     const TlLds lay = tl_lds_layout(a.tlen, RS, OWN, K, WB, la.seg);
     char *lds_c = reinterpret_cast<char *>(lds);
     uint32_t *seg_all = reinterpret_cast<uint32_t *>(lds_c + lay.seg);
-    uint32_t *cellL = reinterpret_cast<uint32_t *>(lds_c + lay.cells);
-    uint32_t *cellN = reinterpret_cast<uint32_t *>(lds_c + lay.cells2);
+    uint32_t *cell0 = reinterpret_cast<uint32_t *>(lds_c + lay.cells);
+    const int cstride = (int)((lay.cells2 - lay.cells) / 4);
     uint8_t *propL = reinterpret_cast<uint8_t *>(lds_c + lay.props);
-    uint8_t *occL = reinterpret_cast<uint8_t *>(lds_c + lay.occ);
+    uint8_t *occ0 = reinterpret_cast<uint8_t *>(lds_c + lay.occ);
+    const int ostride = (int)(lay.occ2 - lay.occ);
     int *misc = reinterpret_cast<int *>(lds_c + lay.misc);
     uint2 *plist = reinterpret_cast<uint2 *>(lds_c + lay.plist);
     W *fieldW = reinterpret_cast<W *>(lds_c + lay.fw), *fieldS = reinterpret_cast<W *>(lds_c + lay.fs);
@@ -88,6 +92,13 @@
         if (t == 0) __hip_atomic_store(la.abort_host, 1u, __ATOMIC_RELAXED, __HIP_MEMORY_SCOPE_SYSTEM);
         return;
     }
+    if (BC == 0 && tl_mirror_ok(a.tlen, L, RS, OWN) == IMG) {
+        if (t == 0) {
+            __hip_atomic_store((tl_gu32 *)la.abort_dev, 1u, __ATOMIC_RELAXED, __HIP_MEMORY_SCOPE_AGENT);
+            __hip_atomic_store(la.abort_host, 1u, __ATOMIC_RELAXED, __HIP_MEMORY_SCOPE_SYSTEM);
+        }
+        return;
+    }
     int n_iter = la.nsteps;
     {
         const unsigned stall = la.abort_dev[1];
@@ -122,8 +133,8 @@
     for (int c = t; c < ncell; c += FU_THREADS) {
         const int s = frame_site(c / K - 1);
         const uint32_t v = cell_e[(unsigned)max(s, 0) * (unsigned)K + (unsigned)(c % K)];
-        cellL[c] = s >= 0 ? v : CELL_EMPTY;
-        if (!K1) cellN[c] = CELL_EMPTY;
+        cell0[c] = s >= 0 ? v : CELL_EMPTY;
+        cell0[cstride + c] = CELL_EMPTY;
     }
 #pragma unroll
     for (int r = 0; r < NOLD; ++r) {
@@ -152,7 +163,7 @@
         }
     }
     const bool wall = BC == 0 && ((x0c + 1 <= Rt) || (L - x1c <= Rt));
-    const bool mirror_ok = 2 * Rt + TS + OWN + 4 < L;
+    constexpr bool HAS_IMG = BC == 0 && IMG, mirror_ok = !HAS_IMG;
     const int sub = lane >> 4, slot = lane & (NSLOT - 1);
     const uint32_t tlen8 = (uint32_t)a.tlen << SH, L8 = (uint32_t)L << SH;
     uint32_t x8[RS];
@@ -182,13 +193,14 @@
     __syncthreads();
     for (int i = t; i < TS + 2; i += FU_THREADS) {
         int n = 0;
-        for (int k = 0; k < K; ++k) n += cellL[i * K + k] != CELL_EMPTY;
-        occL[i] = (uint8_t)n;
+        for (int k = 0; k < K; ++k) n += cell0[i * K + k] != CELL_EMPTY;
+        occ0[i] = (uint8_t)n;
+        occ0[ostride + i] = 0;
     }
     for (int c0 = 0; c0 < ncell; c0 += FU_THREADS) {
         const int c = c0 + t;
         const int pos = K1 ? c - 1 : c / K - 1, k = K1 ? 0 : c - (pos + 1) * K;
-        const uint32_t cw = c < ncell ? cellL[c] : CELL_EMPTY;
+        const uint32_t cw = c < ncell ? cell0[c] : CELL_EMPTY;
         append(cw != CELL_EMPTY && pos >= 0 && pos < nfr, pos, k, cw, misc + 2);
     }
     __syncthreads();
@@ -220,6 +232,8 @@
         const unsigned long long *rec_in = la.xrec + ((size_t)((it + 1) & 1) * a.E * a.ntile + rec_e) * la.rec;
         unsigned long long *rec_out = la.xrec + ((size_t)(it & 1) * a.E * a.ntile + rec_e + tile) * la.rec;
         int *dcount = misc + (it & 1), *pcount = misc + 2 + (it & 1);
+        uint32_t *cellL = cell0 + (it & 1) * cstride, *cellN = cell0 + ((it + 1) & 1) * cstride;
+        uint8_t *occL = occ0 + (it & 1) * ostride, *occN = occ0 + ((it + 1) & 1) * ostride;
         bool gave_up = false;
         const int n0 = *pcount;
         uint2 mine = make_uint2(0u, CELL_EMPTY);
@@ -243,51 +257,24 @@
             gave_up = true;
             return true;
         };
-        auto wait_granule = [&](const unsigned long long *p, bool active) -> uint32_t {
-            unsigned long long x = 0, t_w = 0;
-            for (unsigned spins = 0;;) {
-                if (active) x = tl_load_granule(p);
-                if (!__ballot(active && (uint32_t)(x >> 32) != tag_in)) break;
+        auto wait_granule = [&](const unsigned long long *p, bool active, unsigned long long x) -> uint32_t {
+            unsigned long long t_w = 0;
+            TLSTAMP(8)
+            bool need = active && (uint32_t)(x >> 32) != tag_in;
+            for (unsigned spins = 0; __ballot(need);) {
+                if (need) { x = tl_load_granule(p); need = (uint32_t)(x >> 32) != tag_in; }
+                if (!__ballot(need)) break;
                 if (spin_check(spins, t_w)) break;
             }
+            TLSTAMP(0)
             return (uint32_t)x;
         };
-        if (!first) {
-            unsigned long long t_w = 0;
-            for (unsigned spins = 0;;) {
-                bool bad = false;
-#pragma unroll
-                for (int g = 0; g < TL_NG; ++g) {
-                    bool ok;
-                    const int b = bucket_of(g, ok);
-                    if (ok && (uint32_t)(xg[g] >> 32) != tag_in) {
-                        xg[g] = tl_load_granule(rec_in + (size_t)b * la.rec + slot);
-                        bad |= (uint32_t)(xg[g] >> 32) != tag_in;
-                    }
-                }
-                if (h_act && (uint32_t)(xh >> 32) != tag_in) {
-                    xh = tl_load_granule(rec_in + (size_t)h_nb * la.rec + la.drec + (h_side ? 0 : 3 * K) + h_i);
-                    bad |= (uint32_t)(xh >> 32) != tag_in;
-                }
-                if (!__ballot(bad)) break;
-                if (spin_check(spins, t_w)) break;
-            }
-            if (wave == FU_WAVES - 1 && !gave_up) {
-                const uint32_t v = h_act ? (uint32_t)xh : CELL_EMPTY;
-                const int hs = h_i / K, hk = h_i - hs * K, pos = (h_side ? own_n + 2 : -1) + hs;
-                if (h_act) cellL[(h_side ? (own_n + 3) * K : 0) + h_i] = v;
-                const unsigned long long mo = __ballot(h_act && v != CELL_EMPTY);
-                if (h_i < 3 * K && hk == 0 && h_nb >= 0) occL[pos + 1] = (uint8_t)__popcll((mo >> (h_side * 32 + hs * K)) & ((1ull << K) - 1ull));
-                const bool hp = h_act && v != CELL_EMPTY && pos >= 0 && pos < nfr;
-                const unsigned long long mh = __ballot(hp);
-                if (hp) plist[n0 + __builtin_amdgcn_mbcnt_hi((uint32_t)(mh >> 32), __builtin_amdgcn_mbcnt_lo((uint32_t)mh, 0u))] = make_uint2((uint32_t)pos | ((uint32_t)hk << 16), v);
-                if (lane == 0) misc[4 + (it & 1)] = __popcll(mh);
-            }
-        }
-        TLSTAMP(0)
-        W accP[RS], accM[RS], accF[RS], accWi[RS], accSi[RS];
-#pragma unroll
-        for (int r = 0; r < RS; ++r) accP[r] = accM[r] = accF[r] = accWi[r] = accSi[r] = 0;
+        constexpr int RI = HAS_IMG ? RS : 1;
+        W accP[RS], accM[RS], accF[RS], accWi[RI], accSi[RI];
+#pragma unroll
+        for (int r = 0; r < RS; ++r) accP[r] = accM[r] = accF[r] = 0;
+#pragma unroll
+        for (int r = 0; r < RI; ++r) accWi[r] = accSi[r] = 0;
         uint32_t *shl = seg_all;
         const int CAP = (FU_WAVES * 4 * (SEG + 4) / 4) & ~3;
         unsigned long long *shcnt = reinterpret_cast<unsigned long long *>(misc + 8 + 2 * (it & 1));
@@ -300,8 +287,9 @@
                     if (cls == 0) ts_one_abs<RS, 0, F32>(e1, x8, tb, accP);
                     else if (cls == 1) ts_one_abs<RS, 0, F32>(e1, x8, tb, accM);
                     else if (cls == 2) ts_one_abs<RS, 1, F32>(e1, x8, tb, accF);
-                    else ts_image_group<TAB_LDS, RS, F32>(make_uint4(e1, DEP_NULL | ((uint32_t)x0c + TS_BIAS), DEP_NULL | ((uint32_t)x0c + TS_BIAS), DEP_NULL | ((uint32_t)x0c + TS_BIAS)),
-                                                          x8, tb, table_g, tlen8, L8, accWi, accSi);
+                    else if constexpr (HAS_IMG)
+                        ts_image_group<TAB_LDS, RS, F32>(make_uint4(e1, DEP_NULL | ((uint32_t)x0c + TS_BIAS), DEP_NULL | ((uint32_t)x0c + TS_BIAS), DEP_NULL | ((uint32_t)x0c + TS_BIAS)),
+                                                         x8, tb, table_g, tlen8, L8, accWi, accSi);
                 } else {
                     const uint4 q = make_uint4(e1, DEP_NULL | ((uint32_t)null_site + TS_BIAS), DEP_NULL | ((uint32_t)null_site + TS_BIAS), DEP_NULL | ((uint32_t)null_site + TS_BIAS));
                     if (cls == 0) ts_group<1, TAB_LDS, RS, 0, F32>(q, x8, tb, table_g, tlen8, L8, accP);
@@ -327,15 +315,14 @@
                     en = dep_e[(unsigned)b * (unsigned)a.dcap + min(k0 + slot, (uint32_t)a.dcap - 1u)];
                     valid = k0 + slot < cnt; more = k0 + NSLOT < cnt;
                 } else if (__ballot(active)) {
+                    unsigned long long x = 0;
                     if (page == 0 && j < TL_NG) {
-                        unsigned long long x = xg[0];
+                        x = xg[0];
 #pragma unroll
                         for (int g = 1; g < TL_NG; ++g) if (j == g) x = xg[g];
-                        en = (uint32_t)x;
-                    } else {
-                        en = wait_granule(rb + min(page * NSLOT + slot, la.drec - 1), active);
-                        if (gave_up) break;
                     }
+                    en = wait_granule(rb + min(page * NSLOT + slot, la.drec - 1), active, x);
+                    if (gave_up) break;
                     valid = active && en != DEP_NULL;
                     const unsigned long long mv = __ballot(valid);
                     more = active && ((mv >> (sub * 16 + 15)) & 1ull) && (page + 1) * NSLOT < la.drec;
@@ -389,6 +376,20 @@
                 }
                 active = more;
                 if (!__ballot(active)) break;
+            }
+        }
+        if (!first && wave == FU_WAVES - 1 && !gave_up) {
+            const uint32_t xw = wait_granule(rec_in + (size_t)max(h_nb, 0) * la.rec + la.drec + (h_side ? 0 : 3 * K) + h_i, h_act, xh);
+            if (!gave_up) {
+                const uint32_t v = h_act ? xw : CELL_EMPTY;
+                const int hs = h_i / K, hk = h_i - hs * K, pos = (h_side ? own_n + 2 : -1) + hs;
+                if (h_act) cellL[(h_side ? (own_n + 3) * K : 0) + h_i] = v;
+                const unsigned long long mo = __ballot(h_act && v != CELL_EMPTY);
+                if (h_i < 3 * K && hk == 0 && h_nb >= 0) occL[pos + 1] = (uint8_t)__popcll((mo >> (h_side * 32 + hs * K)) & ((1ull << K) - 1ull));
+                const bool hp = h_act && v != CELL_EMPTY && pos >= 0 && pos < nfr;
+                const unsigned long long mh = __ballot(hp);
+                if (hp) plist[n0 + __builtin_amdgcn_mbcnt_hi((uint32_t)(mh >> 32), __builtin_amdgcn_mbcnt_lo((uint32_t)mh, 0u))] = make_uint2((uint32_t)pos | ((uint32_t)hk << 16), v);
+                if (lane == 0) misc[4 + (it & 1)] = __popcll(mh);
             }
         }
         if (gave_up && lane == 0) misc[TL_ABORT] = 1;
@@ -426,7 +427,7 @@
                 TL_SHARED(2, nF, (ts_group<0, TAB_LDS, RS, 1, F32>(q, x8, tb, table_g, tlen8, L8, accF)))
             }
 #undef TL_SHARED
-            if (nI) {
+            if constexpr (HAS_IMG) if (nI) {
                 const uint32_t nulli = DEP_NULL | ((uint32_t)x0c + TS_BIAS);
                 const uint4 *l4 = reinterpret_cast<const uint4 *>(shl + 3 * CAP);
 #pragma unroll 1
@@ -442,7 +443,8 @@
         TLSTAMP(10)
 #pragma unroll
         for (int r = 0; r < RS; ++r) {
-            const W dw = (accP[r] + accM[r]) + accWi[r], ds = ((accP[r] - accM[r]) + accF[r]) + accSi[r];
+            W dw = accP[r] + accM[r], ds = (accP[r] - accM[r]) + accF[r];
+            if constexpr (HAS_IMG) { dw += accWi[r]; ds += accSi[r]; }
             if (dw != 0) tl_lds_add(&fieldW[r * 64 + lane], dw);
             if (ds != 0) tl_lds_add(&fieldS[r * 64 + lane], ds);
         }
@@ -497,98 +499,95 @@
             R.src[(size_t)e * R.Npad + R.slot_of[(size_t)e * R.N + (c & CELL_ID)]] =
                 (uint32_t)s | DEAD_BIT | ((c & CELL_PLUS) ? SPIN_BIT : 0u) | ((c & CELL_BOUND) ? BOUND_BIT : 0u);
         };
-        uint32_t newc[NOLD];
-        int newn[NOLD];
+        int *pnext = misc + 2 + ((it + 1) & 1);
 #pragma unroll
         for (int r = 0; r < NOLD; ++r) {
-            newc[r] = CELL_EMPTY; newn[r] = 0;
-            const int xi = r * FU_THREADS + t;
-            if (xi < 2 || xi >= 2 + own_n || xi >= TS) continue;
-            const int s = frame_site(xi);
-            if constexpr (K1) {
-                const uint32_t cm2 = cellL[xi - 1], cm1 = cellL[xi], c0 = cellL[xi + 1], cp1 = cellL[xi + 2], cp2 = cellL[xi + 3];
-                const int pm2 = propL[xi - 2] & 7, pm1 = propL[xi - 1] & 7, p0 = propL[xi] & 7, pp1 = propL[xi + 1] & 7, pp2 = xi + 2 < TS ? propL[xi + 2] & 7 : 0;
-                const bool from_l2 = cm2 != CELL_EMPTY && (pm2 == EV_RIGHT || pm2 == EV_FWD);
-                const bool from_l1 = cm1 != CELL_EMPTY && (pm1 == EV_RIGHT || pm1 == EV_FWD);
-                const bool from_r1 = cp1 != CELL_EMPTY && pp1 == EV_LEFT;
-                const bool from_r2 = cp2 != CELL_EMPTY && pp2 == EV_LEFT;
-                uint32_t c = c0;
-                if (c != CELL_EMPTY) {
-                    const int sgn = (c & CELL_PLUS) ? 1 : -1;
-                    uint32_t d0 = 0, d1 = 0;
-                    int nd = 0;
-                    bool stays = true;
-                    if (p0 == EV_LEFT || p0 == EV_RIGHT || p0 == EV_FWD) {
-                        const bool left = p0 == EV_LEFT;
-                        const int rivals = left ? (int)(from_l2 && (cm2 & CELL_ID) < (c & CELL_ID)) + (int)(false)
-                                                : (int)(from_r2 && (cp2 & CELL_ID) < (c & CELL_ID));
-                        if (rivals < 1) {
-                            stays = false;
-                            d0 = deposit(s, -1, -sgn); d1 = deposit(frame_site(left ? xi - 1 : xi + 1), 1, sgn); nd = 2;
+            const int xi = r * FU_THREADS + t, io = xi - 2;
+            const bool mine_site = !(xi < 2 || xi >= 2 + own_n || xi >= TS);
+            uint32_t newc = CELL_EMPTY;
+            int newn = 0;
+            if (mine_site) {
+                const int s = frame_site(xi);
+                if constexpr (K1) {
+                    const uint32_t cm2 = cellL[xi - 1], cm1 = cellL[xi], c0 = cellL[xi + 1], cp1 = cellL[xi + 2], cp2 = cellL[xi + 3];
+                    const int pm2 = propL[xi - 2] & 7, pm1 = propL[xi - 1] & 7, p0 = propL[xi] & 7, pp1 = propL[xi + 1] & 7, pp2 = xi + 2 < TS ? propL[xi + 2] & 7 : 0;
+                    const bool from_l2 = cm2 != CELL_EMPTY && (pm2 == EV_RIGHT || pm2 == EV_FWD);
+                    const bool from_l1 = cm1 != CELL_EMPTY && (pm1 == EV_RIGHT || pm1 == EV_FWD);
+                    const bool from_r1 = cp1 != CELL_EMPTY && pp1 == EV_LEFT;
+                    const bool from_r2 = cp2 != CELL_EMPTY && pp2 == EV_LEFT;
+                    uint32_t c = c0;
+                    if (c != CELL_EMPTY) {
+                        const int sgn = (c & CELL_PLUS) ? 1 : -1;
+                        uint32_t d0 = 0, d1 = 0;
+                        int nd = 0;
+                        bool stays = true;
+                        if (p0 == EV_LEFT || p0 == EV_RIGHT || p0 == EV_FWD) {
+                            const bool left = p0 == EV_LEFT;
+                            const int rivals = left ? (int)(from_l2 && (cm2 & CELL_ID) < (c & CELL_ID)) + (int)(false)
+                                                    : (int)(from_r2 && (cp2 & CELL_ID) < (c & CELL_ID));
+                            if (rivals < 1) {
+                                stays = false;
+                                d0 = deposit(s, -1, -sgn); d1 = deposit(frame_site(left ? xi - 1 : xi + 1), 1, sgn); nd = 2;
+                            }
+                        } else if (p0 == EV_BIND) c |= CELL_BOUND;
+                        else if (p0 == EV_UNBIND) c &= ~CELL_BOUND;
+                        else if (p0 == EV_FLIP) { c ^= CELL_PLUS; d0 = deposit(s, 0, -2 * sgn); nd = 1; }
+                        if (stays) { newc = c; newn = 1; }
+                        if (nd) {
+                            const int kd = atomicAdd(dcount, nd);
+                            if (kd + nd <= a.dcap) { put_deposit(kd, d0); if (nd == 2) put_deposit(kd + 1, d1); }
                         }
-                    } else if (p0 == EV_BIND) c |= CELL_BOUND;
-                    else if (p0 == EV_UNBIND) c &= ~CELL_BOUND;
-                    else if (p0 == EV_FLIP) { c ^= CELL_PLUS; d0 = deposit(s, 0, -2 * sgn); nd = 1; }
-                    if (stays) { newc[r] = c; newn[r] = 1; }
-                    if (nd) {
-                        const int kd = atomicAdd(dcount, nd);
-                        if (kd + nd <= a.dcap) { put_deposit(kd, d0); if (nd == 2) put_deposit(kd + 1, d1); }
                     }
-                }
-                if (from_l1 && !(from_r1 && (cp1 & CELL_ID) < (cm1 & CELL_ID))) { newc[r] = cm1; newn[r] += 1; }
-                if (from_r1 && !(from_l1 && (cm1 & CELL_ID) < (cp1 & CELL_ID))) { newc[r] = cp1; newn[r] += 1; }
-                continue;
-            }
-            uint32_t *outN = cellN + (xi + 1) * K;
-            int n_out = 0;
-            auto emit = [&](uint32_t c) { if (K1) newc[r] = c; else outN[n_out] = c; ++n_out; };
-            for (int k = 0; k < K; ++k) {
-                uint32_t c = cellL[(xi + 1) * K + k];
-                if (c == CELL_EMPTY) continue;
-                const int ev = propL[xi * K + k] & 7, sgn = (c & CELL_PLUS) ? 1 : -1;
-                uint32_t d0 = 0, d1 = 0;
-                int nd = 0;
-                bool stays = true;
-                if (ev == EV_LEFT || ev == EV_RIGHT || ev == EV_FWD) {
-                    const int j = ev == EV_LEFT ? xi - 1 : xi + 1;
-                    if (rank_at(j, c & CELL_ID) < cap_at(j)) {
-                        stays = false;
-                        d0 = deposit(s, -1, -sgn); d1 = deposit(frame_site(j), 1, sgn); nd = 2;
+                    if (from_l1 && !(from_r1 && (cp1 & CELL_ID) < (cm1 & CELL_ID))) { newc = cm1; newn += 1; }
+                    if (from_r1 && !(from_l1 && (cm1 & CELL_ID) < (cp1 & CELL_ID))) { newc = cp1; newn += 1; }
+                    cellN[xi + 1] = newc;
+                } else {
+                    uint32_t *outN = cellN + (xi + 1) * K;
+                    int n_out = 0;
+                    auto emit = [&](uint32_t c) { outN[n_out] = c; ++n_out; };
+                    for (int k = 0; k < K; ++k) {
+                        uint32_t c = cellL[(xi + 1) * K + k];
+                        if (c == CELL_EMPTY) continue;
+                        const int ev = propL[xi * K + k] & 7, sgn = (c & CELL_PLUS) ? 1 : -1;
+                        uint32_t d0 = 0, d1 = 0;
+                        int nd = 0;
+                        bool stays = true;
+                        if (ev == EV_LEFT || ev == EV_RIGHT || ev == EV_FWD) {
+                            const int j = ev == EV_LEFT ? xi - 1 : xi + 1;
+                            if (rank_at(j, c & CELL_ID) < cap_at(j)) {
+                                stays = false;
+                                d0 = deposit(s, -1, -sgn); d1 = deposit(frame_site(j), 1, sgn); nd = 2;
+                            }
+                        } else if (ev == EV_BIND) c |= CELL_BOUND;
+                        else if (ev == EV_UNBIND) c &= ~CELL_BOUND;
+                        else if (ev == EV_FLIP) { c ^= CELL_PLUS; d0 = deposit(s, 0, -2 * sgn); nd = 1; }
+                        else if (ev == EV_EXIT) { stays = false; log_exit(c, s); d0 = deposit(s, -1, -sgn); nd = 1; }
+                        if (stays) emit(c);
+                        if (nd) {
+                            const int kd = atomicAdd(dcount, nd);
+                            if (kd + nd <= a.dcap) { put_deposit(kd, d0); if (nd == 2) put_deposit(kd + 1, d1); }
+                        }
                     }
-                } else if (ev == EV_BIND) c |= CELL_BOUND;
-                else if (ev == EV_UNBIND) c &= ~CELL_BOUND;
-                else if (ev == EV_FLIP) { c ^= CELL_PLUS; d0 = deposit(s, 0, -2 * sgn); nd = 1; }
-                else if (ev == EV_EXIT) { stays = false; log_exit(c, s); d0 = deposit(s, -1, -sgn); nd = 1; }
-                if (stays) emit(c);
-                if (nd) {
-                    const int kd = atomicAdd(dcount, nd);
-                    if (kd + nd <= a.dcap) { put_deposit(kd, d0); if (nd == 2) put_deposit(kd + 1, d1); }
-                }
-            }
-            const int cap = cap_at(xi);
-            for (int k = 0; k < K; ++k) {
-                const uint32_t cl_ = cellL[xi * K + k], cr_ = cellL[(xi + 2) * K + k];
-                const int el = propL[(xi - 1) * K + k] & 7, er = propL[(xi + 1) * K + k] & 7;
-                if (cl_ != CELL_EMPTY && (el == EV_RIGHT || el == EV_FWD) && rank_at(xi, cl_ & CELL_ID) < cap) emit(cl_);
-                if (cr_ != CELL_EMPTY && er == EV_LEFT && rank_at(xi, cr_ & CELL_ID) < cap) emit(cr_);
-            }
-            if (!K1) for (int k = n_out; k < K; ++k) outN[k] = CELL_EMPTY;
-            newn[r] = n_out;
-        }
-        __syncthreads();
-        TLSTAMP(4)
-        const int count = min(*dcount, a.dcap);
-        int *pnext = misc + 2 + ((it + 1) & 1);
-#pragma unroll
-        for (int r = 0; r < NOLD; ++r) {
-            const int xi = r * FU_THREADS + t;
-            const bool mine_site = !(xi < 2 || xi >= 2 + own_n || xi >= TS);
-            const int io = xi - 2;
+                    const int cap = cap_at(xi);
+                    for (int k = 0; k < K; ++k) {
+                        const uint32_t cl_ = cellL[xi * K + k], cr_ = cellL[(xi + 2) * K + k];
+                        const int el = propL[(xi - 1) * K + k] & 7, er = propL[(xi + 1) * K + k] & 7;
+                        if (cl_ != CELL_EMPTY && (el == EV_RIGHT || el == EV_FWD) && rank_at(xi, cl_ & CELL_ID) < cap) emit(cl_);
+                        if (cr_ != CELL_EMPTY && er == EV_LEFT && rank_at(xi, cr_ & CELL_ID) < cap) emit(cr_);
+                    }
+                    for (int k = n_out; k < K; ++k) outN[k] = CELL_EMPTY;
+                    newn = n_out;
+                }
+                occN[xi + 1] = (uint8_t)newn;
+                if (last) {
+                    WS f; f.x = fieldW[xi]; f.y = fieldS[xi];
+                    reinterpret_cast<WS *>(a.ws_out)[(size_t)e * L + (unsigned)s] = f;
+                }
+            }
             for (int k = 0; k < K; ++k) {
                 uint32_t c = CELL_EMPTY;
                 if (mine_site) {
-                    c = K1 ? newc[r] : cellN[(xi + 1) * K + k];
-                    cellL[(xi + 1) * K + k] = c;
+                    c = K1 ? newc : cellN[(xi + 1) * K + k];
                     if (last) cell_o[(unsigned)frame_site(xi) * (unsigned)K + (unsigned)k] = c;
                     else {
                         if (io < 3) tl_store_granule(rec_out + la.drec + io * K + k, tag_out, c);
@@ -597,24 +596,20 @@
                 }
                 if (!last) append(mine_site && c != CELL_EMPTY, xi, k, c, pnext);
             }
-            if (mine_site) {
-                occL[xi + 1] = (uint8_t)newn[r];
-                if (last) {
-                    WS f; f.x = fieldW[xi]; f.y = fieldS[xi];
-                    reinterpret_cast<WS *>(a.ws_out)[(size_t)e * L + (unsigned)frame_site(xi)] = f;
-                }
-            }
-        }
-        if (!last && t < NSLOT) {
-            const int idx = count + t;
-            if (idx < (count / NSLOT + 1) * NSLOT && idx < la.drec) tl_store_granule(rec_out + idx, tag_out, DEP_NULL);
-        }
-        for (int i = t; i < (TS * K + 3) / 4; i += FU_THREADS) reinterpret_cast<uint32_t *>(propL)[i] = 0u;
+        }
         if (t == 0) {
             misc[(it + 1) & 1] = 0;
             misc[2 + (it & 1)] = 0; misc[4 + (it & 1)] = 0;
             misc[8 + 2 * (it & 1)] = 0; misc[9 + 2 * (it & 1)] = 0;
-            if (last) {
+        }
+        TLSTAMP(4)
+        __syncthreads();
+        if (t < NSLOT) {
+            const int count = min(*dcount, a.dcap);
+            if (!last) {
+                const int idx = count + t;
+                if (idx < (count / NSLOT + 1) * NSLOT && idx < la.drec) tl_store_granule(rec_out + idx, tag_out, DEP_NULL);
+            } else if (t == 0) {
                 a.dcnt_out[(size_t)e * a.ntile + tile] = (uint32_t)count;
                 if (tile == 0 && e == 0) a.stepw[(a.par + la.nsteps) & 1] = la.step0 + (unsigned long long)la.nsteps;
             }
@@ -630,7 +625,6 @@
             xh = h_act ? tl_load_granule(rn + (size_t)h_nb * la.rec + la.drec + (h_side ? 0 : 3 * K) + h_i) : 0ull;
         }
         TLSTAMP(5)
-        __syncthreads();
     }
 #ifdef APS_LOOP_STAMPS
     if (lane == 0 && tile < 512 && e == 0) {
```

Result: faster. 8.493 billion particle-steps/s, median of 6 (+3.2%).
